# jacky121298/3DAL_PyTorch

Measured on AMD Instinct MI355X. Metric: object-crops/sec through static+dynamic refinement heads, higher is better.
Workload: dtype f32; 1 GPU; StaticModelOneBoxEst forward+decode, 4096 crops x 1024 pts per GPU, fp32 (BASELINE.json configs[1]); items_per_gpu=4096, points_per_item=1024, sampler=device, parallelism=single GPU

## Files before the change

3dal_pytorch_amd/_hip.py:

```python
import ctypes as C
import os

import numpy as np
import torch

_HERE = os.path.dirname(os.path.abspath(__file__))
LIB_PATH = os.path.join(_HERE, "lib3dal_hip.so")

OK, EINVAL, EWORKSPACE, EHIP = 0, -1, -2, -3
F32, BF16, F16, F16X3 = 0, 1, 2, 3
DTYPES = {"fp32": F32, "bf16": BF16, "fp16": F16, "f16x3": F16X3}
HEAD_INS_SEG, HEAD_STATIC_BOX_EST, HEAD_POINT_EMB, HEAD_BOX_EMB, HEAD_DYNAMIC_BOX_EST = range(5)
SAMPLER_DEVICE, SAMPLER_CHOICE = 0, 1
PHASE_SEG, PHASE_BOX, PHASE_ALL = 1, 2, 3

vp = C.c_void_p


class Layer(C.Structure):
    _fields_ = [("weight", vp), ("bias", vp), ("bn_weight", vp), ("bn_bias", vp), ("bn_mean", vp),
                ("bn_var", vp), ("c_in", C.c_int32), ("c_out", C.c_int32)]


class PackItem(C.Structure):
# ... 246 lines not shown
    _fields_ = [("c_in", C.c_int32), ("n_shared", C.c_int32), ("n_cls", C.c_int32), ("n_reg", C.c_int32), ("shared", _i3),
                ("cls", _i3), ("reg", _i3), ("num_class", C.c_int32), ("code_size", C.c_int32)]


class RoiHeadArgs(C.Structure):
    _fields_ = [("shape", RoiShape), ("packed", vp), ("B", C.c_int64), ("M", C.c_int64), ("num_point", C.c_int32), ("C", C.c_int32),
                ("T", C.c_int32), ("box_cols", C.c_int32), ("K", C.c_int64), ("keep_stride", C.c_int64), ("boxes", vp), ("scores", vp),
                ("labels", vp), ("keep", vp), ("keep_count", vp), ("seg_offsets", vp), ("label_base", C.c_int32 * ROI_MAX_TASKS),
                ("bev", Map), ("H", C.c_int64), ("W", C.c_int64), ("pc_start", _f2), ("voxel_size", _f2), ("out_stride", C.c_float),
                ("rois", vp), ("roi_scores", vp), ("roi_features", vp), ("out_boxes", vp), ("out_scores", vp), ("out_labels", vp),
                ("out_counts", vp), ("out_features", vp), ("box_preds", vp), ("cls_preds", vp), ("status", vp), ("workspace", vp),
                ("workspace_bytes", C.c_size_t)]


ROI_NO_SAMPLE = 8192
ROI_CLS_SCORE = {"roi_iou": 0, "cls": 1}
ROI_TRAIN_MAX_M, ROI_TRAIN_MAX_R, ROI_TRAIN_MAX_G = 512, 512, 1024


class RoiTargetsArgs(C.Structure):
    _fields_ = [("B", C.c_int64), ("M", C.c_int64), ("R", C.c_int64), ("G", C.c_int64), ("code_size", C.c_int32),
                ("reserved0", C.c_int32), ("T", C.c_int32), ("reserved", C.c_int32), ("K", C.c_int64), ("keep_stride", C.c_int64),
                ("boxes", vp), ("scores", vp), ("labels", vp), ("keep", vp), ("keep_count", vp), ("seg_offsets", vp),
                ("label_base", C.c_int32 * ROI_MAX_TASKS), ("rois", vp), ("roi_scores", vp), ("roi_labels", vp), ("gt", vp),
                ("draws", vp), ("fg_per_image", C.c_int32), ("cls_score_type", C.c_int32), ("reg_fg_thresh", C.c_float),
                ("cls_fg_thresh", C.c_float), ("cls_bg_thresh", C.c_float), ("cls_bg_thresh_lo", C.c_float),
                ("cls_thresh_span", C.c_float), ("reserved2", C.c_float), ("hard_bg_ratio", C.c_double), ("slot", vp), ("sample", vp),
                ("out_rois", vp), ("out_labels", vp), ("out_scores", vp), ("gt_iou", vp), ("gt_src", vp), ("reg_valid", vp),
                ("cls_labels", vp), ("gt_of_rois", vp), ("out_boxes", vp), ("status", vp)]


CENTER_OVERFLOW = 16384
CENTER_MAX_OBJS, CENTER_MAX_CLASSES, CENTER_MAX_COLS = 1024, 64, 10
_pT = vp * ROI_MAX_TASKS


class CenterTargetsArgs(C.Structure):
    _fields_ = [("B", C.c_int64), ("G", C.c_int64), ("H", C.c_int64), ("W", C.c_int64), ("T", C.c_int32), ("max_objs", C.c_int32),
                ("num_class", C.c_int32 * ROI_MAX_TASKS), ("gt", vp), ("pc_start", _f2), ("voxel_size", _f2),
                ("out_size_factor", C.c_float), ("min_radius", C.c_int32), ("gaussian_overlap", C.c_double), ("hm", _pT),
                ("anno_box", _pT), ("ind", _pT), ("mask", _pT), ("cat", _pT), ("status", vp)]


class CenterLossArgs(C.Structure):
    _fields_ = [("B", C.c_int64), ("H", C.c_int64), ("W", C.c_int64), ("C", C.c_int32), ("n_cols", C.c_int32), ("max_objs", C.c_int32),
                ("reserved", C.c_int32), ("hm", Map), ("reg", Map), ("height", Map), ("dim", Map), ("rot", Map), ("vel", Map),
                ("target_hm", vp), ("anno_box", vp), ("ind", vp), ("mask", vp), ("cat", vp),
                ("code_weights", C.c_float * CENTER_MAX_COLS), ("weight", C.c_float), ("reserved2", C.c_float), ("out", vp),
                ("grad", vp), ("workspace", vp), ("workspace_bytes", C.c_size_t)]


AUG_TOO_MANY, AUG_OVERFLOW, AUG_BAD_ROW = 32768, 65536, 131072
AUG_MAX_BOXES, AUG_MAX_CAND = 1024, 64


class GtPasteArgs(C.Structure):
    _fields_ = [("B", C.c_int64), ("max_gt", C.c_int32), ("max_cand", C.c_int32), ("gt_boxes", vp), ("gt_classes", vp),
                ("gt_counts", vp), ("cand_boxes", vp), ("cand_group", vp), ("cand_counts", vp), ("accept", vp), ("coll", vp),
                ("status", vp)]


class AugmentPointsArgs(C.Structure):
    _fields_ = [("B", C.c_int64), ("n", C.c_int64), ("n_scene", C.c_int64), ("db_rows", C.c_int64), ("F", C.c_int32),
                ("transform", C.c_int32), ("max_cand", C.c_int64), ("scene", vp), ("scene_offsets", vp), ("db_points", vp),
                ("out_offsets", vp), ("cand_counts", vp), ("cand_seg_start", vp), ("cand_rows", vp), ("cand_db_row", vp),
                ("cand_boxes", vp), ("accept", vp), ("keys", vp), ("xform", vp), ("out", vp), ("status", vp),
                ("max_workgroups", C.c_int64), ("workspace", vp), ("workspace_bytes", C.c_size_t)]


class AugmentBoxesArgs(C.Structure):
    _fields_ = [("B", C.c_int64), ("max_gt", C.c_int32), ("max_cand", C.c_int32), ("max_objs", C.c_int32), ("n_classes", C.c_int32),
                ("transform", C.c_int32), ("reserved", C.c_int32), ("gt_boxes", vp), ("gt_classes", vp), ("gt_counts", vp),
                ("cand_boxes", vp), ("cand_classes", vp), ("cand_counts", vp), ("accept", vp), ("xform", vp),
                ("range", C.c_float * 4), ("out", vp), ("out_count", vp), ("status", vp)]


_i, _i64, _u64, _sz = C.c_int, C.c_int64, C.c_uint64, C.c_size_t
SIGNATURES = {
    "dal3_version": (_i, []),
    "dal3_last_error": (C.c_char_p, []),
    "dal3_mean_size": (C.POINTER(C.c_float), []),
    "dal3_pack_weights": (_i, [_i, C.POINTER(Layer), _i, _i, vp, C.POINTER(_sz), vp]),
    "dal3_ins_seg_workspace_bytes": (_sz, [_i]),
    "dal3_ins_seg_forward": (_i, [vp, _i, _i, BCN, _i, _i, vp, vp, vp, vp, _sz, vp]),
    "dal3_ins_seg_encode": (_i, [vp, _i, _i, BCN, _i, _i, vp, vp]),
    "dal3_ins_seg_global_bias": (_i, [vp, _i, vp, _i, vp, vp]),
    "dal3_ins_seg_decode": (_i, [vp, _i, _i, BCN, _i, _i, vp, vp, vp, vp]),
    "dal3_gather_workspace_bytes": (_sz, [_i, _i]),
    "dal3_segment_counts": (_i, [vp, _i, _i, vp, vp]),
    "dal3_mask_compact_sample": (_i, [vp, BCN, _i, _i, _i, _i, _i, vp, _u64, _i64, vp, vp, vp, vp, _sz, vp]),
    "dal3_mask_compact_sample_step": (_i, [vp, BCN, _i, _i, _i, _i, _u64, vp, _i64, vp, vp, vp, vp, _sz, vp]),
    "dal3_point_head_workspace_bytes": (_sz, [_i]),
    "dal3_point_head_forward": (_i, [_i, vp, _i, BCN, _i, _i, vp, _i64, vp, _sz, vp]),
    "dal3_point_head_pool_workspace_bytes": (_sz, [_i, _i]),
    "dal3_point_head_screen_min_tiles": (_i, []),
    "dal3_point_head_screen_stride": (_i, []),
    "dal3_point_head_pool": (_i, [_i, vp, _i, BCN, _i, _i, vp, vp, vp, _sz, vp]),
    "dal3_dynamic_box_est_forward": (_i, [vp, vp, _i, vp, vp, _sz, vp]),
    "dal3_decode_boxes": (_i, [vp, _i, vp, _i64, _i, vp, _i64, vp, _i64, vp, vp, vp, vp, vp]),
    "dal3_recenter_rotz": (_i, [vp, _i, _i, vp, vp, vp, vp, vp, vp, vp]),
    "dal3_static_crop_prep": (_i, [vp, vp, vp, vp, vp, _i, _i, _u64, _i64, vp, vp, vp]),
    "dal3_dynamic_item_prep": (_i, [vp, vp, vp, vp, vp, vp, vp, vp, _i, _i, _i, _i, _u64, _i64, vp, vp, vp, vp]),
    "dal3_writeback_boxes": (_i, [vp, vp, vp, vp, vp, vp, vp, vp, vp, _i, _i64, vp, vp, vp]),
    "dal3_static_crop_labels": (_i, [vp, vp, vp, vp, _i, _i, _u64, _i64, vp, vp, vp]),
    "dal3_dynamic_item_labels": (_i, [vp, vp, vp, vp, vp, vp, vp, _i, _i, _i, _u64, _i64, vp, vp, vp, vp, vp]),
    "dal3_points_in_boxes": (_i, [vp, _i, _i64, _i64, vp, _i, _i, vp, vp]),
    "dal3_box_iou_pairwise": (_i, [vp, _i64, vp, _i64, _i, vp, vp, vp]),
    "dal3_box_iou_paired": (_i, [vp, vp, _i64, _i, vp, vp, vp]),
    "dal3_box_estimation_metrics": (_i, [C.POINTER(BoxMetricArgs), vp]),
    "dal3_track_workspace_bytes": (_sz, [_i64, _i64, _i64]),
    "dal3_track": (_i, [C.POINTER(TrackArgs), vp]),
    "dal3_track_match_workspace_bytes": (_sz, [_i64]),
    "dal3_track_match": (_i, [C.POINTER(TrackMatchArgs), vp]),
    "dal3_group_workspace_bytes": (_sz, [_i64, _i64]),
    "dal3_group_by_key": (_i, [C.POINTER(GroupArgs), vp]),
    "dal3_track_features": (_i, [C.POINTER(TrackFeatureArgs), vp]),
    "dal3_gt_table": (_i, [C.POINTER(GtTableArgs), vp]),
    "dal3_motion_classify_workspace_bytes": (_sz, [_i64]),
    "dal3_motion_classify": (_i, [C.POINTER(MotionClassifyArgs), vp]),
    "dal3_score_workspace_bytes": (_sz, [_i64]),
    "dal3_score_tracks": (_i, [C.POINTER(ScoreArgs), vp]),
    "dal3_best_gt_iou": (_i, [C.POINTER(BestGtArgs), vp]),
    "dal3_nms_workspace_bytes": (_sz, [_i64, _i]),
    "dal3_nms": (_i, [C.POINTER(NmsArgs), vp]),
    "dal3_center_decode_workspace_bytes": (_sz, [_i64, _i64, _i64]),
    "dal3_center_decode": (_i, [C.POINTER(CenterDecodeArgs), vp]),
    "dal3_center_decode_flip4_workspace_bytes": (_sz, [_i64, _i64, _i64]),
    "dal3_center_decode_flip4": (_i, [C.POINTER(CenterDecodeFlip4Args), vp]),
    "dal3_flip4_points": (_i, [vp, _i64, C.c_int32, vp, _i64, vp, vp, _i64, vp]),
    "dal3_voxelize_workspace_bytes": (_sz, [_i64, _i64]),
    "dal3_voxelize": (_i, [C.POINTER(VoxelizeArgs), vp]),
    "dal3_pillar_pack": (_i, [C.POINTER(Layer), _i, _i, C.c_double, vp, vp]),
    "dal3_pillar_features": (_i, [C.POINTER(PillarFeatureArgs), vp]),
    "dal3_pillar_scatter": (_i, [vp, vp, _i64, vp, _i, vp, _i64, _i64, _i64, vp]),
    "dal3_voxel_mean": (_i, [vp, vp, _i64, vp, _i, _i, vp, vp]),
    "dal3_conv2d_pack_floats": (_sz, [_i, _i, _i]),
    "dal3_conv2d_pack": (_i, [C.POINTER(Layer), _i, C.c_double, vp, vp]),
    "dal3_conv2d": (_i, [C.POINTER(Conv2dArgs), vp]),
    "dal3_sp_sort_workspace_bytes": (_sz, [_i64]),
    "dal3_sp_sort": (_i, [C.POINTER(SpSortArgs), vp]),
    "dal3_sp_downsample_workspace_bytes": (_sz, [_i64, _i]),
    "dal3_sp_downsample": (_i, [C.POINTER(SpDownsampleArgs), vp]),
    "dal3_sp_table": (_i, [C.POINTER(SpTableArgs), vp]),
    "dal3_sp_conv_pack_floats": (_sz, [_i, _i, _i]),
    "dal3_sp_conv_pack": (_i, [C.POINTER(Layer), _i, C.c_double, vp, vp, vp]),
    "dal3_sp_conv": (_i, [C.POINTER(SpConvArgs), vp]),
    "dal3_sp_table_transposed": (_i, [C.POINTER(SpTableTransposedArgs), vp]),
    "dal3_sp_wgrad_workspace_bytes": (_sz, [_i, _i, _i, _i64]),
    "dal3_sp_wgrad": (_i, [C.POINTER(SpWgradArgs), vp]),
    "dal3_bev_gather": (_i, [C.POINTER(BevGatherArgs), vp]),
    "dal3_box_points": (_i, [vp, _i64, _i, _i, vp, vp]),
    "dal3_roi_pack_floats": (_sz, [C.POINTER(RoiShape)]),
    "dal3_roi_pack": (_i, [C.POINTER(RoiShape), C.POINTER(Layer), _i, C.POINTER(C.c_double), vp, vp]),
    "dal3_roi_head_workspace_bytes": (_sz, [_i64, _i64, _i, _i, _i]),
    "dal3_roi_head": (_i, [C.POINTER(RoiHeadArgs), vp]),
    "dal3_roi_post": (_i, [vp, vp, vp, _i64, _i, vp, vp, vp]),
    "dal3_roi_targets": (_i, [C.POINTER(RoiTargetsArgs), vp]),
    "dal3_roi_loss": (_i, [vp, vp, _i64, _i, vp, vp, vp, C.POINTER(C.c_float), C.c_float, C.c_float, vp, vp, vp, vp]),
    "dal3_center_targets": (_i, [C.POINTER(CenterTargetsArgs), vp]),
    "dal3_center_loss_workspace_bytes": (_sz, [_i64, _i64, _i64, _i64]),
    "dal3_center_loss": (_i, [C.POINTER(CenterLossArgs), vp]),
    "dal3_gt_paste_select": (_i, [C.POINTER(GtPasteArgs), vp]),
    "dal3_augment_points_workspace_bytes": (_sz, [_i64, _i64]),
    "dal3_augment_points": (_i, [C.POINTER(AugmentPointsArgs), vp]),
    "dal3_augment_boxes": (_i, [C.POINTER(AugmentBoxesArgs), vp]),
    "dal3_crop_workspace_bytes": (_sz, [_i64, _i64]),
# ... 60 lines not shown
    "dal3_tr_wgrad_x3": (_i, [vp, _i64, vp, _i64, vp, vp, _i, vp, _i64, _i, _i, vp, _sz, vp, vp]),
    "dal3_tr_segmax": (_i, [vp, _i64, _i64, _i, vp, vp, vp, vp, _i64, vp, _sz, vp]),
    "dal3_tr_act_dropout": (_i, [vp, _i64, _i, _i64, vp, vp, _i, vp, _i64, _u64, vp, C.c_float, vp, _i64, vp]),
    "dal3_tr_linear_pool_workspace_bytes": (_sz, [_i, _i, _i64]),
    "dal3_tr_linear_pool": (_i, [vp, _i64, _i, _i64, vp, vp, _i, vp, _i64, vp, vp, vp, _i64, _i, vp, vp, vp, _sz, vp]),
    "dal3_tr_linear_pool_x3": (_i, [vp, _i64, _i, _i64, vp, vp, _i, vp, _i64, vp, vp, vp, _i64, _i, vp, vp, vp, _sz, vp]),
    "dal3_tr_linear_pool_x3_ok": (_i, [_i64, _i, _i64, _i]),
    "dal3_tr_segsum": (_i, [vp, _i64, _i64, _i, vp, _i64, vp]),
    "dal3_maxpool_n": (_i, [vp, _i64, _i64, vp, vp]),
    "dal3_maxpool_n_dtype": (_i, [vp, _i, _i64, _i64, vp, vp]),
    "dal3_shared_mlp_layer": (_i, [C.POINTER(Layer), _i, BCN, _i, _i, vp, vp, _sz, vp]),
    "dal3_shared_mlp_layer_workspace_bytes": (_sz, [_i, _i]),
    "dal3_static_workspace_bytes": (_sz, [_i, _i, _i]),
    "dal3_static_forward": (_i, [C.POINTER(StaticArgs), _i, vp]),
    "dal3_dynamic_workspace_bytes": (_sz, [_i, _i, _i]),
    "dal3_dynamic_forward": (_i, [C.POINTER(DynamicArgs), _i, vp]),
}

_lib = None


def lib():
    global _lib
    if _lib is None:
        if not os.path.exists(LIB_PATH):
            raise RuntimeError(
                f"{LIB_PATH} is missing: build the HIP library first "
                "(`make -C 3dal_pytorch_amd/csrc` or __graft_entry__.build()). "
                "There is no CPU/eager fallback for the eval-mode forward.")
        handle = C.CDLL(LIB_PATH)
        for name, (res, args) in SIGNATURES.items():
            fn = getattr(handle, name)
            fn.restype = res
            fn.argtypes = args
        from . import arch
        lib_mean = [handle.dal3_mean_size()[i] for i in range(9)]
        want = [C.c_float(v).value for row in arch.MEAN_SIZE for v in row]
        if lib_mean != want:
            raise RuntimeError(f"lib3dal_hip.so was built with MEAN_SIZE {lib_mean}, arch.MEAN_SIZE is {want}: rebuild the library")
        _lib = handle
    return _lib


def check(rc):
    if rc != OK:
        raise RuntimeError(f"lib3dal_hip error {rc}: {lib().dal3_last_error().decode()}")


def stream():
    return vp(torch.cuda.current_stream().cuda_stream)


def ptr(t):
    return vp(t.data_ptr()) if t is not None else vp(None)


def require_gpu(t, what):
    if not t.is_cuda:
        raise RuntimeError(
            f"{what} lives on {t.device}: the eval-mode forward runs only on an MI355X through "
            "lib3dal_hip.so (no CPU fallback). Move the model and its inputs to the GPU.")


def workspace(nbytes, device):
    return torch.empty(max(int(nbytes), 8), dtype=torch.uint8, device=device)


def host_offsets(offsets, n, name, sized_by, count):
    if torch.is_tensor(offsets):
        if offsets.is_cuda:
            raise TypeError(f"{name} must be on the host (a list, an array or a CPU tensor): {sized_by} from it, and "
                            "reading a device tensor back would be the synchronisation this call avoids")
        offsets = offsets.numpy()
    off = np.ascontiguousarray(np.asarray(offsets, dtype=np.int64).reshape(-1))
    if off.size < 1:
        raise ValueError(f"{name} needs {count} + 1 entries")
    if off[0] < 0 or off[-1] > n or np.any(np.diff(off) < 0):
        raise ValueError(f"{name} must be non-decreasing within [0, {n}]")
    return off


STORAGE = {torch.float32: F32, torch.bfloat16: BF16, torch.float16: F16}
BCN_NO_SMALL_JOB_KERNELS, BCN_NO_WORKLIST, BCN_NO_LDS_SAMPLER = 1, 2, 4
DISPATCH_FLAGS = 0


def bcn(t):
    assert t.dim() == 3 and t.dtype in STORAGE
    sb, sc, sn = t.stride()
    return BCN(ptr(t), sb, sc, sn, STORAGE[t.dtype], DISPATCH_FLAGS)


def layer_struct(conv, bn):
    w = conv.weight
    c_in, c_out = getattr(conv, "in_channels", w.shape[1]), getattr(conv, "out_channels", w.shape[0])
    if not w.is_contiguous() or w.dtype != torch.float32:
        raise RuntimeError("weights must be contiguous fp32")
    L = Layer(ptr(w), ptr(conv.bias), None, None, None, None, c_in, c_out)
    if bn is not None:
        L.bn_weight, L.bn_bias = ptr(bn.weight), ptr(bn.bias)
        L.bn_mean, L.bn_var = ptr(bn.running_mean), ptr(bn.running_var)
    return L


def fold_layer_struct(conv, bn, what="the layer's parameters"):
    ts = [conv.weight] + ([conv.bias] if conv.bias is not None else [])
    if bn is not None:
        ts += [bn.weight, bn.bias, bn.running_mean, bn.running_var]
    for t in ts:
        require_gpu(t, what)
        if t.dtype != torch.float32 or not t.is_contiguous():
            raise RuntimeError("weights must be contiguous fp32")
    return layer_struct(conv, bn)


F16_MAX = 65504.0


def check_f16x3_range(pairs):
    with torch.no_grad():
        worst = None
        for conv, bn in pairs:
            w = conv.weight.detach().reshape(conv.weight.shape[0], -1).abs().amax(1)
            if bn is not None:
                w = w * (bn.weight.detach() / torch.sqrt(bn.running_var.detach() + 1e-5)).abs()
            m = w.max()
            worst = m if worst is None else torch.maximum(worst, m)
        if worst is not None and not float(worst) < F16_MAX:
            raise ValueError(f"precision 'f16x3': a folded weight of magnitude {float(worst):.3g} is beyond fp16's range "
                             f"({F16_MAX:g}); this head cannot run on the f16x3 kernels (use precision 'fp32')")


def pack(head_kind, pairs, device, dtype=F32):
    if dtype == F16X3:
        check_f16x3_range(pairs)
    arr = (Layer * len(pairs))(*[layer_struct(c, b) for c, b in pairs])
    need = _sz(0)
    check(lib().dal3_pack_weights(head_kind, arr, len(pairs), dtype, None, C.byref(need), None))
    buf = torch.empty(need.value, dtype=torch.uint8, device=device)
    assert buf.data_ptr() % 256 == 0
    check(lib().dal3_pack_weights(head_kind, arr, len(pairs), dtype, ptr(buf), C.byref(need), stream()))
    return buf
```

3dal_pytorch_amd/csrc/dal3_api.hip:

```cpp
#include <stdarg.h>
#include <stdio.h>
#include <string.h>

#include "dal3_block.h"
#include "dal3_kernels.h"
#include "dal3_lp.h"

static thread_local char g_err[512] = "";

static int fail(int code, const char* fmt, ...) {
    va_list ap;
    va_start(ap, fmt);
    vsnprintf(g_err, sizeof(g_err), fmt, ap);
    va_end(ap);
    return code;
}

#define HIP_TRY(expr)                                                                           \
    do {                                                                                        \
        hipError_t e_ = (expr);                                                                 \
        if (e_ != hipSuccess) return fail(DAL3_EHIP, "%s: %s", #expr, hipGetErrorString(e_)); \
    } while (0)
#define TRY(expr)               \
    do {                        \
        int r_ = (expr);        \
        if (r_ != 0) return r_; \
    } while (0)

extern "C" int dal3_version(void) { return DAL3_VERSION; }
extern "C" const float* dal3_mean_size(void) {
    static const float v[9] = {DAL3_MEAN_SIZE_VALUES};
    return v;
}
extern "C" const char* dal3_last_error(void) { return g_err; }

static inline size_t al(size_t floats) { return (floats + 63) & ~(size_t)63; }

struct Cursor {
    const float* base;
    size_t off;
    const float* take(size_t floats) {
        const float* p = base ? base + off : nullptr;
        off += al(floats);
        return p;
    }
    const f32x4* take4(size_t floats) { return reinterpret_cast<const f32x4*>(take(floats)); }
};

static InsSegW ins_seg_walk(Cursor& c) {
    InsSegW w;
    w.w1 = c.take(2 * 2 * 64);
    w.b1 = c.take(64);    w.b2 = c.take(64);    w.b3 = c.take(64);    w.b4 = c.take(128);   w.b5 = c.take(1024);
    w.dw1g = c.take(512 * 1024);
    w.db1 = c.take(512);  w.db2 = c.take(256);  w.db3 = c.take(128);  w.db4 = c.take(128);
    w.dw5 = c.take(2 * 128);
    w.db5 = c.take(32);
    w.enc_stream = c.take4((size_t)ENC_FRAGS * 256);
    w.dec_stream = c.take4((size_t)DEC_FRAGS * 256);
    w.lat_stream = c.take4((size_t)LAT_FRAGS * 256);
    w.w5row = c.take((size_t)1024 * 128);
    w.w5h = c.take4((size_t)32 * 4 * 2 * 256);
    w.scr_pq = c.take(2 * 1024);
    w.scr_flag = reinterpret_cast<const int32_t*>(c.take(64));
    w.dw2c = c.take((size_t)512 * 256);
    w.dw3c = c.take((size_t)256 * 128);
    w.dw4c = c.take((size_t)128 * 128);
    w.dec_flag = reinterpret_cast<const int32_t*>(c.take(64));
    return w;
}

size_t ins_seg_packed_floats(int) {
    Cursor c{nullptr, 0};
    ins_seg_walk(c);
    return c.off + DAL3_BLOB_TAIL_FLOATS;
}
InsSegW ins_seg_view(const float* base, int) {
    Cursor c{base, 0};
    return ins_seg_walk(c);
}

void point_head_dims(int head_kind, int* c_in, int* ks, int c[4], int* n_fc, int fc_in[3], int fc_out[3]) {
    switch (head_kind) {
        case DAL3_HEAD_STATIC_BOX_EST:
            *c_in = 3; *ks = 2; c[0] = 128; c[1] = 128; c[2] = 256; c[3] = 512; *n_fc = 3;
            fc_in[0] = 512; fc_out[0] = 512; fc_in[1] = 512; fc_out[1] = 256; fc_in[2] = 256; fc_out[2] = 39;
            break;
        case DAL3_HEAD_POINT_EMB:
            *c_in = 4; *ks = 2; c[0] = 64; c[1] = 128; c[2] = 256; c[3] = 512; *n_fc = 2;
            fc_in[0] = 512; fc_out[0] = 512; fc_in[1] = 512; fc_out[1] = 256; fc_in[2] = 0; fc_out[2] = 0;
            break;
        default:
            *c_in = 8; *ks = 4; c[0] = 64; c[1] = 64; c[2] = 128; c[3] = 512; *n_fc = 2;
            fc_in[0] = 512; fc_out[0] = 128; fc_in[1] = 128; fc_out[1] = 128; fc_in[2] = 0; fc_out[2] = 0;
            break;
    }
}

static PointHeadW point_head_walk(Cursor& cur, int head_kind) {
    int c_in, ks, c[4], n_fc, fi[3], fo[3];
    point_head_dims(head_kind, &c_in, &ks, c, &n_fc, fi, fo);
    PointHeadW w;
    w.w1 = cur.take((size_t)(c[0] / 32) * ks * 64);
    w.b1 = cur.take(c[0]);    w.b2 = cur.take(c[1]);    w.b3 = cur.take(c[2]);    w.b4 = cur.take(c[3]);
    w.stream = cur.take4(((size_t)(c[1] / 32) * (c[0] / 32) + (size_t)(c[2] / 32) * (c[1] / 32) +
                          (size_t)(c[3] / 32) * (c[2] / 32)) * 1024);
    w.fc.n = n_fc;
    for (int i = 0; i < 3; ++i) {
        w.fc.c_in[i] = fi[i];
        w.fc.c_out[i] = fo[i];
        w.fc.relu[i] = !(head_kind == DAL3_HEAD_STATIC_BOX_EST && i == 2);
        w.fc.w[i] = i < n_fc ? cur.take((size_t)fi[i] * fo[i]) : nullptr;
        w.fc.b[i] = i < n_fc ? cur.take((fo[i] + 31) / 32 * 32) : nullptr;
    }
    const bool scr = c[2] == 256 && c[3] == 512;
    w.w4row = scr ? cur.take((size_t)512 * 256) : nullptr;
    w.w4h = scr ? cur.take4((size_t)16 * 8 * 2 * 256) : nullptr;
    w.scr_pq = scr ? cur.take(2 * 512) : nullptr;
    w.scr_flag = scr ? reinterpret_cast<const int32_t*>(cur.take(64)) : nullptr;
    return w;
}
size_t point_head_packed_floats(int head_kind) {
    Cursor c{nullptr, 0};
    point_head_walk(c, head_kind);
    return c.off + DAL3_BLOB_TAIL_FLOATS;
}
PointHeadW point_head_view(const float* base, int head_kind) {
    Cursor c{base, 0};
    return point_head_walk(c, head_kind);
}

static const int kDynFcIn[3] = {384, 128, 128}, kDynFcOut[3] = {128, 128, 39};
static FcW fc_head_walk(Cursor& cur) {
    FcW f;
    f.n = 3;
    for (int i = 0; i < 3; ++i) {
        f.c_in[i] = kDynFcIn[i];
        f.c_out[i] = kDynFcOut[i];
        f.relu[i] = i < 2;
        f.w[i] = cur.take((size_t)kDynFcIn[i] * kDynFcOut[i]);
        f.b[i] = cur.take((kDynFcOut[i] + 31) / 32 * 32);
    }
    return f;
}
size_t fc_head_packed_floats() {
    Cursor c{nullptr, 0};
    fc_head_walk(c);
    return c.off;
}
FcW fc_head_view(const float* base) {
// ... 187 lines not shown
            HIP_TRY(launch_pack_weight(L[0], PACK_FIRST, 0, c_in, 2, 2, mut(w.w1), s));
            HIP_TRY(launch_pack_bias(L[0], mut(w.b1), s));
            HIP_TRY(launch_pack_bias(L[1], be, s));
            HIP_TRY(launch_pack_bias(L[2], be + 64, s));
            HIP_TRY(launch_pack_bias(L[3], be + 128, s));
            HIP_TRY(launch_pack_bias(L[4], be + 256, s));
            HIP_TRY(launch_pack_bias(L[1], bd, s));
            HIP_TRY(launch_pack_bias(L[6], bd + 64, s));
            HIP_TRY(launch_pack_bias(L[7], bd + 320, s));
            HIP_TRY(launch_pack_bias(L[8], bd + 448, s));
            HIP_TRY(launch_pack_bias(L[9], bd + 576, s));
            HIP_TRY(launch_pack_weight(L[5], PACK_ROWMAJOR, 64, 1024, 0, 0, mut(w.dw1g), s));
            HIP_TRY(launch_pack_bias(L[5], mut(w.db1), s));
            HIP_TRY(launch_pack_weight_x3(L[1], 0, 0, 64, 2, 2, enc, s));
            HIP_TRY(launch_pack_weight_x3(L[2], 0, 0, 64, 2, 2, enc + 16 * F, s));
            HIP_TRY(launch_pack_weight_x3(L[3], 0, 0, 64, 4, 2, enc + 32 * F, s));
            HIP_TRY(launch_pack_weight_x3(L[4], 0, 0, 128, 32, 4, enc + 64 * F, s));
            HIP_TRY(launch_pack_weight_x3(L[1], 0, 0, 64, 2, 2, dec, s));
            HIP_TRY(launch_pack_weight_x3(L[5], 0, 0, 64, 16, 2, dec, s, 2, 16 * F, 24 * F, 40 * F));
            HIP_TRY(launch_pack_weight_x3(L[6], 1, 0, 512, 8, 16, dec, s, 8, 32 * F, 72 * F, 40 * F, 624 * F));
            HIP_TRY(launch_pack_weight_x3(L[7], 0, 0, 256, 4, 8, dec + 656 * F, s));
            HIP_TRY(launch_pack_weight_x3(L[8], 0, 0, 128, 4, 4, dec + 784 * F, s));
            HIP_TRY(launch_pack_weight_x3(L[9], 0, 0, 128, 1, 4, dec + 848 * F, s));
            return 0;
        }
        if (lp) {
            const InsSegLpW w = ins_seg_lp_view(packed_dev);
            uint16_t* enc = const_cast<uint16_t*>(w.enc_stream);
            uint16_t* dec = const_cast<uint16_t*>(w.dec_stream);
            float* be = mut(w.bias_enc);
            float* bd = mut(w.bias_dec);
            const int64_t F = 512;
            HIP_TRY(launch_pack_weight(L[0], PACK_FIRST, 0, c_in, 2, 2, mut(w.w1), s));
            HIP_TRY(launch_pack_bias(L[0], mut(w.b1), s));
            HIP_TRY(launch_pack_bias(L[1], be, s));
            HIP_TRY(launch_pack_bias(L[2], be + 64, s));
            HIP_TRY(launch_pack_bias(L[3], be + 128, s));
            HIP_TRY(launch_pack_bias(L[4], be + 256, s));
            HIP_TRY(launch_pack_bias(L[1], bd, s));
            HIP_TRY(launch_pack_bias(L[6], bd + 64, s));
            HIP_TRY(launch_pack_bias(L[7], bd + 320, s));
            HIP_TRY(launch_pack_bias(L[8], bd + 448, s));
            HIP_TRY(launch_pack_weight(L[9], PACK_ROWMAJOR, 0, 128, 0, 0, bd + 576, s));
            HIP_TRY(launch_pack_bias(L[9], bd + 832, s));
            HIP_TRY(launch_pack_weight(L[5], PACK_ROWMAJOR, 64, 1024, 0, 0, mut(w.dw1g), s));
            HIP_TRY(launch_pack_bias(L[5], mut(w.db1), s));
            HIP_TRY(launch_pack_weight_lp(L[1], dtype, 0, 0, 64, 2, 2, enc, s));
            HIP_TRY(launch_pack_weight_lp(L[2], dtype, 0, 0, 64, 2, 2, enc + 8 * F, s));
            HIP_TRY(launch_pack_weight_lp(L[3], dtype, 0, 0, 64, 4, 2, enc + 16 * F, s));
            HIP_TRY(launch_pack_weight_lp(L[4], dtype, 0, 0, 128, 32, 4, enc + 32 * F, s));
            HIP_TRY(launch_pack_weight_lp(L[1], dtype, 0, 0, 64, 2, 2, dec, s));
            HIP_TRY(launch_pack_weight_lp(L[5], dtype, 0, 0, 64, 16, 2, dec, s, 2, 8 * F, 40 * F, 20 * F));
            HIP_TRY(launch_pack_weight_lp(L[6], dtype, 1, 0, 512, 8, 16, dec, s, 8, 44 * F, 64 * F, 20 * F));
            HIP_TRY(launch_pack_weight_lp(L[7], dtype, 0, 0, 256, 4, 8, dec, s, 16, 360 * F, 400 * F, 40 * F));
            HIP_TRY(launch_pack_weight_lp(L[8], dtype, 0, 0, 128, 4, 4, dec + 440 * F, s));
            HIP_TRY(launch_pack_weight_lp(L[9], dtype, 0, 0, 128, 1, 4, dec + 472 * F, s));
            return 0;
        }
        InsSegW w = ins_seg_view(base, c_in);
        HIP_TRY(launch_pack_weight(L[0], PACK_FIRST, 0, c_in, 2, 2, mut(w.w1), s));
        HIP_TRY(launch_pack_bias(L[0], mut(w.b1), s));
        TRY(pack_frag(L[1], PACK_FRAG_MT_MAJOR, 0, 64, w.enc_stream, ENC_W2, w.b2, s));
        TRY(pack_frag(L[2], PACK_FRAG_MT_MAJOR, 0, 64, w.enc_stream, ENC_W3, w.b3, s));
        TRY(pack_frag(L[3], PACK_FRAG_MT_MAJOR, 0, 64, w.enc_stream, ENC_W4, w.b4, s));
        TRY(pack_frag(L[4], PACK_FRAG_MT_MAJOR, 0, 128, w.enc_stream, ENC_W5, w.b5, s));
        TRY(pack_frag(L[1], PACK_FRAG_MT_MAJOR, 0, 64, w.dec_stream, DEC_W2, nullptr, s));
        TRY(pack_frag(L[5], PACK_FRAG_MT_MAJOR, 0, 64, w.dec_stream, DEC_MIX, w.db1, s,  2,
                      0, 8 * 256, 40 * 256));
        HIP_TRY(launch_pack_weight(L[5], PACK_ROWMAJOR, 64, 1024, 0, 0, mut(w.dw1g), s));
        TRY(pack_frag(L[6], PACK_FRAG_KT_MAJOR, 0, 512, w.dec_stream, DEC_MIX, w.db2, s,  8,
                      16 * 256, 56 * 256, 40 * 256));
        TRY(pack_frag(L[7], PACK_FRAG_MT_MAJOR, 0, 256, w.dec_stream, DEC_W3, w.db3, s));
        TRY(pack_frag(L[8], PACK_FRAG_MT_MAJOR, 0, 128, w.dec_stream, DEC_W4, w.db4, s));
        TRY(pack_frag(L[5], PACK_FRAG_MT_MAJOR, 0, 64, w.lat_stream, LAT_W1A, nullptr, s));
        TRY(pack_frag(L[6], PACK_FRAG_MT_MAJOR, 0, 512, w.lat_stream, LAT_W2, nullptr, s));
        HIP_TRY(launch_pack_weight(L[9], PACK_ROWMAJOR, 0, 128, 0, 0, mut(w.dw5), s));
        HIP_TRY(launch_pack_bias(L[9], mut(w.db5), s));
        HIP_TRY(launch_pack_weight(L[4], PACK_ROWMAJOR, 0, 128, 0, 0, mut(w.w5row), s));
        HIP_TRY(launch_pack_weight_lp(L[4], DAL3_F16, 0, 0, 128, 32, 4, reinterpret_cast<uint16_t*>(mut(w.w5h)), s));
        HIP_TRY(launch_pack_enc_screen(L[4], mut(w.scr_pq), reinterpret_cast<int32_t*>(mut(w.scr_flag)), s));
        HIP_TRY(launch_pack_dec_sparse(L[6], w.db2, mut(w.dw2c), reinterpret_cast<int32_t*>(const_cast<int32_t*>(w.dec_flag)), s));
        HIP_TRY(launch_pack_dec_queue(L[7], 256, w.db3, mut(w.dw3c), reinterpret_cast<int32_t*>(const_cast<int32_t*>(w.dec_flag)), s));
        HIP_TRY(launch_pack_dec_queue(L[8], 128, w.db4, mut(w.dw4c), reinterpret_cast<int32_t*>(const_cast<int32_t*>(w.dec_flag)), s));
        return 0;
    }
    if (head_kind == DAL3_HEAD_DYNAMIC_BOX_EST) {
        if (n_layers != 3) return fail(DAL3_EINVAL, "dynamic box_est expects 3 layers, got %d", n_layers);
        return pack_fc(L, fc_head_view(base), s);
    }
    int c_in, ks, c[4], n_fc, fi[3], fo[3];
    point_head_dims(head_kind, &c_in, &ks, c, &n_fc, fi, fo);
    if (n_layers != 4 + n_fc) return fail(DAL3_EINVAL, "head %d expects %d layers, got %d", head_kind, 4 + n_fc, n_layers);
    TRY(check_layer(L[0], c_in, c[0], "conv1"));
    for (int i = 1; i < 4; ++i) TRY(check_layer(L[i], c[i - 1], c[i], "conv"));
    if (x3) {
        const PointHeadX3W w = point_head_x3_view(packed_dev, head_kind);
        HIP_TRY(launch_pack_weight(L[0], PACK_FIRST, 0, c_in, c[0] / 32, ks, mut(w.w1), s));
        HIP_TRY(launch_pack_bias(L[0], mut(w.b1), s));
        HIP_TRY(launch_pack_bias(L[1], mut(w.bias), s));
        HIP_TRY(launch_pack_bias(L[2], mut(w.bias) + c[1], s));
        HIP_TRY(launch_pack_bias(L[3], mut(w.bias) + c[1] + c[2], s));
        uint16_t* st = const_cast<uint16_t*>(w.stream);
        int64_t off = 0;
        for (int l = 1; l < 4; ++l) {
            const int kt = c[l - 1] / 32, mt = c[l] / 32;
            HIP_TRY(launch_pack_weight_x3(L[l], 0, 0, c[l - 1], mt, kt, st + off, s));
            off += (int64_t)mt * kt * 2048;
        }
        return pack_fc(L + 4, w.fc, s);
    }
    if (lp) {
        const PointHeadLpW w = point_head_lp_view(packed_dev, head_kind);
        HIP_TRY(launch_pack_weight(L[0], PACK_FIRST, 0, c_in, c[0] / 32, ks, mut(w.w1), s));
        HIP_TRY(launch_pack_bias(L[0], mut(w.b1), s));
        HIP_TRY(launch_pack_bias(L[1], mut(w.bias), s));
        HIP_TRY(launch_pack_bias(L[2], mut(w.bias) + c[1], s));
        HIP_TRY(launch_pack_bias(L[3], mut(w.bias) + c[1] + c[2], s));
        uint16_t* st = const_cast<uint16_t*>(w.stream);
        const int64_t SEGE = (int64_t)LP_HEAD_SEG * 512;
        int seg = 0;
        for (int l = 1; l < 4; ++l) {
            const int kt = c[l - 1] / 32, mt = c[l] / 32, tps = lp_tps(kt, mt);
            HIP_TRY(launch_pack_weight_lp(L[l], dtype, 0, 0, c[l - 1], mt, kt, st, s, tps * kt, seg * SEGE,
                                          (seg + 1) * SEGE, SEGE));
            seg += mt / tps;
        }
        return pack_fc(L + 4, w.fc, s);
    }
    PointHeadW w = point_head_view(base, head_kind);
    HIP_TRY(launch_pack_weight(L[0], PACK_FIRST, 0, c_in, c[0] / 32, ks, mut(w.w1), s));
    HIP_TRY(launch_pack_bias(L[0], mut(w.b1), s));
    const int f3 = (c[1] / 32) * (c[0] / 32) * 4, f4 = f3 + (c[2] / 32) * (c[1] / 32) * 4;
    TRY(pack_frag(L[1], PACK_FRAG_MT_MAJOR, 0, c[0], w.stream, 0, w.b2, s));
    TRY(pack_frag(L[2], PACK_FRAG_MT_MAJOR, 0, c[1], w.stream, f3, w.b3, s));
    TRY(pack_frag(L[3], PACK_FRAG_MT_MAJOR, 0, c[2], w.stream, f4, w.b4, s));
    if (w.w4row) {
        HIP_TRY(launch_pack_weight(L[3], PACK_ROWMAJOR, 0, 256, 0, 0, mut(w.w4row), s));
        HIP_TRY(launch_pack_weight_lp(L[3], DAL3_F16, 0, 0, 256, 16, 8, reinterpret_cast<uint16_t*>(mut(w.w4h)), s));
        HIP_TRY(launch_pack_head_screen(L[3], mut(w.scr_pq), reinterpret_cast<int32_t*>(mut(w.scr_flag)), s));
    }
    return pack_fc(L + 4, w.fc, s);
}

static BCN to_bcn(const dal3_bcn& t) { return BCN{t.data, t.stride_b, t.stride_c, t.stride_n, t.dtype, t.flags}; }

static int check_bcn(const dal3_bcn& t, const char* what) {
    if (!t.data) return fail(DAL3_EINVAL, "%s: null data pointer", what);
    if (t.stride_n <= 0 || t.stride_c <= 0) return fail(DAL3_EINVAL, "%s: strides must be positive", what);
    if (t.dtype != DAL3_F32 && t.dtype != DAL3_BF16 && t.dtype != DAL3_F16)
        return fail(DAL3_EINVAL, "%s: storage dtype %d is none of DAL3_F32 / DAL3_BF16 / DAL3_F16", what, t.dtype);
    if (t.dtype != DAL3_F32 && (reinterpret_cast<uintptr_t>(t.data) & 1)) return fail(DAL3_EINVAL, "%s: 16-bit data must be 2-byte aligned", what);
    if (t.flags & ~(DAL3_BCN_NO_SMALL_JOB_KERNELS | DAL3_BCN_NO_WORKLIST | DAL3_BCN_NO_LDS_SAMPLER)) return fail(DAL3_EINVAL, "%s: unknown bits in flags (%d)", what, t.flags);
    return 0;
}

static int check_extent(int64_t B, int64_t N, const char* what) {
    if (B <= 0 || N <= 0) return fail(DAL3_EINVAL, "%s: B and N must be positive (B=%lld N=%lld)", what, (long long)B, (long long)N);
    if (B > DAL3_MAX_ITEMS) return fail(DAL3_EINVAL, "%s: B=%lld items exceed DAL3_MAX_ITEMS (%d)", what, (long long)B, DAL3_MAX_ITEMS);
    if (N > DAL3_MAX_POINTS_PER_ITEM)
        return fail(DAL3_EINVAL, "%s: N=%lld points per item exceed DAL3_MAX_POINTS_PER_ITEM (%d)", what, (long long)N, DAL3_MAX_POINTS_PER_ITEM);
    if (B * ((N + 31) / 32) > (int64_t)DAL3_MAX_TILES)
        return fail(DAL3_EINVAL, "%s: B=%lld x N=%lld is %lld 32-point tiles, more than DAL3_MAX_TILES (%d): split the batch", what,
                    (long long)B, (long long)N, (long long)(B * ((N + 31) / 32)), DAL3_MAX_TILES);
    return 0;
}

struct InsSegWs { float* g; float* gb; };
static InsSegWs carve_ins_seg(Carver& c, int B) {
    InsSegWs w;
    w.g = c.take<float>((size_t)B * 1024);
    w.gb = c.take<float>((size_t)B * 512);
    return w;
}
extern "C" size_t dal3_ins_seg_workspace_bytes(int B) {
    Carver c(nullptr, 0);
    carve_ins_seg(c, B);
    return c.off;
}

static int check_dtype(int dtype) {
    if (dtype != DAL3_F32 && dtype != DAL3_BF16 && dtype != DAL3_F16 && dtype != DAL3_F16X3)
        return fail(DAL3_EINVAL, "unknown dtype %d", dtype);
    return 0;
}

static int ins_seg_run(const void* packed, int dtype, int c_in, const dal3_bcn& pts, int B, int N, float* logits,
                       uint8_t* mask, float* global_feat_out, const InsSegWs& ws, hipStream_t s) {
    TRY(check_dtype(dtype));
    if (!packed || !logits || !mask) return fail(DAL3_EINVAL, "ins_seg: null pointer");
    TRY(check_extent(B, N, "ins_seg"));
    if (c_in != 3 && c_in != 4) return fail(DAL3_EINVAL, "ins_seg: c_in must be 3 or 4");
    TRY(check_bcn(pts, "pts"));
    const BCN x = to_bcn(pts);
    HIP_TRY(launch_nonfinite_rows(x, B, N, c_in, ws.g, 1024, s));
    if (dtype == DAL3_F32) {
        const InsSegW w = ins_seg_view(static_cast<const float*>(packed), c_in);
        HIP_TRY(launch_ins_seg_encode(w, x, c_in, B, N, ws.g, s));
        HIP_TRY(launch_fc(w.dw1g, w.db1, ws.g, 1024, ws.gb, 512, B, 1024, 512, 0, s));
        HIP_TRY(launch_ins_seg_decode(w, x, c_in, B, N, ws.gb, logits, mask, s));
    } else if (dtype == DAL3_F16X3) {
        const InsSegX3W w = ins_seg_x3_view(packed);
        HIP_TRY(launch_ins_seg_encode_x3(w, x, c_in, B, N, ws.g, s));
        HIP_TRY(launch_fc(w.dw1g, w.db1, ws.g, 1024, ws.gb, 512, B, 1024, 512, 0, s));
        HIP_TRY(launch_ins_seg_decode_x3(w, x, c_in, B, N, ws.gb, logits, mask, s));
    } else {
        const InsSegLpW w = ins_seg_lp_view(packed);
        HIP_TRY(launch_ins_seg_encode_lp(dtype, w, x, c_in, B, N, ws.g, s));
        HIP_TRY(launch_fc(w.dw1g, w.db1, ws.g, 1024, ws.gb, 512, B, 1024, 512, 0, s));
        HIP_TRY(launch_ins_seg_decode_lp(dtype, w, x, c_in, B, N, ws.gb, logits, mask, s));
    }
    if (global_feat_out)
        HIP_TRY(hipMemcpyAsync(global_feat_out, ws.g, (size_t)B * 1024 * sizeof(float), hipMemcpyDeviceToDevice, s));
    return 0;
}

extern "C" int dal3_ins_seg_forward(const void* packed, int dtype, int c_in, dal3_bcn pts, int B, int N, float* logits,
                                    uint8_t* mask, float* global_feat_out, void* workspace, size_t workspace_bytes,
                                    dal3_stream stream) {
    if (!workspace) return fail(DAL3_EINVAL, "ins_seg: workspace is NULL");
    TRY(check_extent(B, N, "ins_seg"));
    Carver c(workspace, workspace_bytes);
    const InsSegWs ws = carve_ins_seg(c, B);
    if (!c.ok) return fail(DAL3_EWORKSPACE, "ins_seg: workspace needs %zu bytes, got %zu", c.off, workspace_bytes);
    return ins_seg_run(packed, dtype, c_in, pts, B, N, logits, mask, global_feat_out, ws, static_cast<hipStream_t>(stream));
}

extern "C" int dal3_ins_seg_encode(const void* packed, int dtype, int c_in, dal3_bcn pts, int B, int N,
                                   float* global_feat, dal3_stream stream) {
    TRY(check_dtype(dtype));
    if (!packed || !global_feat || (c_in != 3 && c_in != 4)) return fail(DAL3_EINVAL, "ins_seg_encode: bad argument");
    TRY(check_extent(B, N, "ins_seg_encode"));
    TRY(check_bcn(pts, "pts"));
    hipStream_t s = static_cast<hipStream_t>(stream);
    if (dtype == DAL3_F32)
        HIP_TRY(launch_ins_seg_encode(ins_seg_view(static_cast<const float*>(packed), c_in), to_bcn(pts), c_in, B, N,
                                      global_feat, s));
    else if (dtype == DAL3_F16X3)
        HIP_TRY(launch_ins_seg_encode_x3(ins_seg_x3_view(packed), to_bcn(pts), c_in, B, N, global_feat, s));
    else
        HIP_TRY(launch_ins_seg_encode_lp(dtype, ins_seg_lp_view(packed), to_bcn(pts), c_in, B, N, global_feat, s));
    return 0;
}

extern "C" int dal3_ins_seg_global_bias(const void* packed, int dtype, const float* global_feat, int B, float* gbias,
                                        dal3_stream stream) {
    TRY(check_dtype(dtype));
    if (!packed || !global_feat || !gbias) return fail(DAL3_EINVAL, "ins_seg_global_bias: bad argument");
    TRY(check_extent(B, 1, "ins_seg_global_bias"));
    const float* dw1g = dtype == DAL3_F32 ? ins_seg_view(static_cast<const float*>(packed), 3).dw1g
                        : dtype == DAL3_F16X3 ? ins_seg_x3_view(packed).dw1g : ins_seg_lp_view(packed).dw1g;
    const float* db1 = dtype == DAL3_F32 ? ins_seg_view(static_cast<const float*>(packed), 3).db1
                       : dtype == DAL3_F16X3 ? ins_seg_x3_view(packed).db1 : ins_seg_lp_view(packed).db1;
    HIP_TRY(launch_fc(dw1g, db1, global_feat, 1024, gbias, 512, B, 1024, 512, 0, static_cast<hipStream_t>(stream)));
    return 0;
}

extern "C" int dal3_ins_seg_decode(const void* packed, int dtype, int c_in, dal3_bcn pts, int B, int N,
                                   const float* gbias, float* logits, uint8_t* mask, dal3_stream stream) {
    TRY(check_dtype(dtype));
    if (!packed || !gbias || !logits || !mask || (c_in != 3 && c_in != 4)) return fail(DAL3_EINVAL, "ins_seg_decode: bad argument");
    TRY(check_extent(B, N, "ins_seg_decode"));
    TRY(check_bcn(pts, "pts"));
    hipStream_t s = static_cast<hipStream_t>(stream);
    if (dtype == DAL3_F32)
        HIP_TRY(launch_ins_seg_decode(ins_seg_view(static_cast<const float*>(packed), c_in), to_bcn(pts), c_in, B, N,
                                      gbias, logits, mask, s));
    else if (dtype == DAL3_F16X3)
        HIP_TRY(launch_ins_seg_decode_x3(ins_seg_x3_view(packed), to_bcn(pts), c_in, B, N, gbias, logits, mask, s));
    else
        HIP_TRY(launch_ins_seg_decode_lp(dtype, ins_seg_lp_view(packed), to_bcn(pts), c_in, B, N, gbias, logits, mask, s));
    return 0;
}

extern "C" size_t dal3_gather_workspace_bytes(int B, int N) {
    Carver c(nullptr, 0);
    c.take<int32_t>((size_t)B * N);
    return c.off;
}

extern "C" int dal3_segment_counts(const uint8_t* mask, int B, int N, int32_t* counts, dal3_stream stream) {
    if (!mask || !counts) return fail(DAL3_EINVAL, "segment_counts: bad argument");
    TRY(check_extent(B, N, "segment_counts"));
// ... 1985 lines not shown
```

3dal_pytorch_amd/csrc/dal3_enc_screen.hip:

```cpp
#include "dal3_device.h"
#include "dal3_kernels.h"
#include "dal3_lp.h"
#include "dal3_screen.h"

#ifndef SCR_CAP
#define SCR_CAP 1024
#endif
#define SCR_XLD 132
#define SCR_STAGE_LD 36
#ifndef SCR_DEPTH
#define SCR_DEPTH 2
#endif
#define SCR_XMAX_BITS 0x476A6000
#ifndef DAL3_SCR_A_STRIDE
#define DAL3_SCR_A_STRIDE 4
#endif
static_assert(DAL3_SCR_A_STRIDE >= 1, "pass A's stride over the wave-slots");

#ifdef DAL3_SCREEN_COUNT
__device__ unsigned long long g_scr_count[8];
extern "C" int dal3_debug_screen_counts(unsigned long long* out, int reset) {
    hipError_t e = hipMemcpyFromSymbol(out, HIP_SYMBOL(g_scr_count), sizeof(g_scr_count));
    if (e == hipSuccess && reset) {
        unsigned long long z[8] = {};
        e = hipMemcpyToSymbol(HIP_SYMBOL(g_scr_count), z, sizeof(z));
    }
    return (int)e;
}
#define SCR_COUNT(k, v)                                           \
    do {                                                          \
        if (lane == 0) atomicAdd(&g_scr_count[k], (unsigned long long)(v)); \
    } while (0)
#else
#define SCR_COUNT(k, v)
#endif

template <int PASS, int T>
__global__ __launch_bounds__(64 * DAL3_WG_WAVES) void ins_seg_encode_screen_kernel(InsSegW w, BCN pts, int c_in, int n_pts,
                                                                                  int tiles_per_item, float* __restrict__ g) {
    const int lane = threadIdx.x & 63;
    const int wave = threadIdx.x >> 6;
    const int h = lane >> 5;
    const int64_t b = blockIdx.x / tiles_per_item;
    const int n0 = ((blockIdx.x % tiles_per_item) * DAL3_WG_WAVES + wave) * (PASS == 0 ? DAL3_SCR_A_STRIDE : 1) * (32 * T);
    __shared__ float s_b5[1024];
    __shared__ int s_max[1024];
    __shared__ f32x2 s_pq[1024];
    __shared__ float s_g[PASS == 1 ? 1024 : 1];
    __shared__ __attribute__((aligned(16))) float s_x[PASS == 1 ? DAL3_WG_WAVES * 32 * SCR_XLD : 4];
    __shared__ uint32_t s_list[PASS == 1 ? DAL3_WG_WAVES * T * SCR_CAP : 1];
    __shared__ __attribute__((aligned(16))) uint32_t s_stage[PASS == 1 ? DAL3_WG_WAVES * 64 * SCR_STAGE_LD : 4];
    int* gi = reinterpret_cast<int*>(g + b * 1024);
    static_assert(20 * 1024 + DAL3_WG_WAVES * (32 * SCR_XLD * 4 + T * SCR_CAP * 4 + 64 * SCR_STAGE_LD * 4) <= 160 * 1024,
                  "pass B's LDS exceeds a CU's 160 KiB: lower SCR_CAP, DAL3_WG_WAVES or DAL3_ENC_T");
    static_assert(32 * 64 <= 64 * SCR_STAGE_LD, "a wave's stage holds the hit words of conv5's 32 blocks");
    if (PASS == 0 && *w.scr_flag != 0) return;
    for (int i = threadIdx.x; i < 1024; i += 64 * DAL3_WG_WAVES) {
        s_b5[i] = w.b5[i];
        s_max[i] = 0;
        s_pq[i] = reinterpret_cast<const f32x2*>(w.scr_pq)[i];
        if (PASS == 1) s_g[i] = __int_as_float(__hip_atomic_load(gi + i, __ATOMIC_RELAXED, __HIP_MEMORY_SCOPE_AGENT));
    }
    __syncthreads();
    if (n0 < n_pts) {
        WRing<DAL3_PF> ring;
        ring.init(w.enc_stream, lane);
        f32x16 bias = tile_from_channels(w.b2, h);
        float in[T][2];
        load_points<2, T>(pts, b, n0, n_pts, c_in, in, lane);
        f32x16 x1[T][2], x2[T][2], x3[T][2], x4[T][4];
        first_layer<2, 2, T>(w.w1, w.b1, in, x1, lane);
        mlp_layer_ring<2, 2, T>(ring, w.b2, w.b3, bias, x1, x2, lane);
        mlp_layer_ring<2, 2, T>(ring, w.b3, w.b4, bias, x2, x3, lane);
        mlp_layer_ring<2, 4, T>(ring, w.b4, w.b4, bias, x3, x4, lane);
        SCR_COUNT(0, 1);

        int xm = 0;
#pragma unroll
        for (int j = 0; j < T; ++j) {
#pragma unroll
            for (int kt = 0; kt < 4; ++kt) {
#pragma unroll
                for (int r = 0; r < 16; ++r) {
                    const int v = __float_as_int(x4[j][kt][r]);
                    xm = v > xm ? v : xm;
                }
            }
        }
        const bool dense = *w.scr_flag != 0 || __builtin_amdgcn_ballot_w64(xm > SCR_XMAX_BITS) != 0;
        if (dense) {
            SCR_COUNT(1, 1);
            if (PASS == 1) conv_max_layer<4, T>(ring, s_b5, x4, reinterpret_cast<float*>(s_max), 32, lane);
        } else {
            float x2max = 0.0f;
#pragma unroll
            for (int j = 0; j < T; ++j) {
                float ss = 0.0f;
#pragma unroll
                for (int kt = 0; kt < 4; ++kt) {
#pragma unroll
                    for (int r = 0; r < 16; ++r) ss = fmaf(x4[j][kt][r], x4[j][kt][r], ss);
                }
                ss += __shfl_xor(ss, 32);
                x2max = __builtin_fmaxf(x2max, ss);
            }
#pragma unroll
            for (int d = 16; d >= 1; d >>= 1) x2max = __builtin_fmaxf(x2max, __shfl_xor(x2max, d));
            const float X = sqrtf(x2max) * (1.0f + 0x1p-16f);

            ActTile<FP16> xh[T][4];
#pragma unroll
            for (int j = 0; j < T; ++j) {
#pragma unroll
                for (int kt = 0; kt < 4; ++kt) xh[j][kt] = pack_relu<FP16>(x4[j][kt]);
            }

            uint32_t* const list = s_list + (PASS == 1 ? wave * T * SCR_CAP : 0);
            uint32_t* const stage = s_stage + (PASS == 1 ? wave * 64 * SCR_STAGE_LD : 0);
            ScreenHits<T> hits;
            hits.init();

            auto block_const = [&](int mt) -> float {
                const int c = 32 * mt + (lane & 31);
                const f32x2 pq = s_pq[c];
                float E = fmaf(X, pq[0], pq[1]);
                E = fmaf(E, 0x1p-20f, E);
                if (PASS == 0) return E;
                const float G = s_g[c], bb = s_b5[c];
                if (bits_nonfinite(G)) return 3.0e38f;
                return (G - bb) - fmaf(__builtin_fabsf(G) + __builtin_fabsf(bb), 0x1p-22f, E);
            };
            static_assert(16 * T <= 32, "one hit bit per (tile, register) in a 32-bit word");
            float m = 0.0f;
            uint32_t hb = 0;
            auto ep_slice = [&](const f32x16 (&acc)[T], int i, float k) {
#pragma unroll
                for (int rr = 0; rr < 2; ++rr) {
#pragma unroll
                    for (int j = 0; j < T; ++j) {
                        const int r = 2 * i + rr;
                        if (PASS == 0)
                            m = (r == 0 && j == 0) ? acc[0][0] : __builtin_fmaxf(m, acc[j][r]);
                        else
                            hb = scr_push_hit(hb, acc[j][r], k);
                    }
                }
            };
            auto ep_finish = [&](int mt, float k) {
                const int c = 32 * mt + (lane & 31);
                if (PASS == 0) {
                    m = __builtin_fmaxf(m, __shfl_xor(m, 32));
                    const float y = m - fmaf(__builtin_fabsf(m), 0x1p-22f, k);
                    int bits = __float_as_int(y + s_b5[c]);
                    bits = bits > 0 ? bits : 0;
                    if (lane < 32 && bits > 0) atomicMax(&s_max[c], bits);
// ... 3 lines not shown
            };

            WRing<8> r16;
            r16.init(w.w5h, lane);
            auto mm = [&](f32x16 (&acc)[T], auto side) {
#pragma unroll
                for (int j = 0; j < T; ++j) acc[j] = f32x16{};
#pragma unroll
                for (int i = 0; i < 8; ++i) {
                    const f16x8_t a = __builtin_bit_cast(f16x8_t, r16.slot[i]);
                    r16.slot[i] = r16.fetch();
#pragma unroll
                    for (int j = 0; j < T; ++j) acc[j] = FP16::mfma(xh[j][i >> 1].k[i & 1], a, acc[j]);
                    DAL3_SCHED_FENCE();
                    side(i);
                    DAL3_SCHED_FENCE();
                }
            };
            f32x16 accA[T], accB[T];
            float kA = block_const(0), kB;
            mm(accA, NoSide());
            int mt = 1;
            for (; mt + 1 < 32; mt += 2) {
                kB = block_const(mt);
                mm(accB, [&](int i) { ep_slice(accA, i, kA); });
                ep_finish(mt - 1, kA);
                kA = block_const(mt + 1);
                mm(accA, [&](int i) { ep_slice(accB, i, kB); });
                ep_finish(mt, kB);
            }
            kB = block_const(mt);
            mm(accB, [&](int i) { ep_slice(accA, i, kA); });
            ep_finish(mt - 1, kA);
#pragma unroll
            for (int i = 0; i < 8; ++i) ep_slice(accB, i, kB);
            ep_finish(mt, kB);

            if (PASS == 1) {
                uint32_t cnt[T];
                const bool overflow = scr_build_lists<T, 32, SCR_CAP>(stage, list, hits, cnt, lane);
#pragma unroll
                for (int j = 0; j < T; ++j) SCR_COUNT(3, cnt[j]);
                if (overflow) {
                    SCR_COUNT(2, 1);
                    WRing<DAL3_PF> r32;
                    r32.init(w.enc_stream + ENC_W5 * 64, lane);
                    conv_max_layer<4, T>(r32, s_b5, x4, reinterpret_cast<float*>(s_max), 32, lane);
                } else {
                    float* const xw = s_x + wave * 32 * SCR_XLD;
#pragma unroll
                    for (int j = 0; j < T; ++j) {
                        __builtin_amdgcn_wave_barrier();
#pragma unroll
                        for (int kt = 0; kt < 4; ++kt) {
#pragma unroll
                            for (int q = 0; q < 4; ++q) {
                                f32x4 v;
                                v[0] = x4[j][kt][4 * q + 0];
                                v[1] = x4[j][kt][4 * q + 1];
                                v[2] = x4[j][kt][4 * q + 2];
                                v[3] = x4[j][kt][4 * q + 3];
                                *reinterpret_cast<f32x4*>(xw + (lane & 31) * SCR_XLD + 32 * kt + 8 * q + 4 * h) = v;
                            }
                        }
                        __builtin_amdgcn_wave_barrier();
                        SCR_COUNT(4, (cnt[j] + 63) / 64);
                        scr_recompute<32, 4, SCR_DEPTH, true>(
                            w.w5row, 128, list + j * SCR_CAP, cnt[j], xw, SCR_XLD, stage, lane, [](uint32_t, bool) { return 0.0f; },
                            [&](float a, int c, uint32_t, bool live) {
                                int bits = __float_as_int(a + s_b5[c]);
                                bits = bits > 0 ? bits : 0;
                                if (live && bits > 0) atomicMax(&s_max[c], bits);
                            });
                    }
                }
            }
        }
    }
    __syncthreads();
    for (int c = threadIdx.x; c < 1024; c += 64 * DAL3_WG_WAVES) {
        const int v = s_max[c];
        if (v > 0) atomicMax(gi + c, v);
    }
}

hipError_t launch_ins_seg_encode_screen(const InsSegW& w, BCN pts, int c_in, int B, int N, float* g, hipStream_t s) {
    constexpr int T = DAL3_ENC_T;
    const int tpi = (N + 32 * DAL3_WG_WAVES * T - 1) / (32 * DAL3_WG_WAVES * T);
    const int slots = (N + 32 * T - 1) / (32 * T);
    const int tpi_a = ((slots + DAL3_SCR_A_STRIDE - 1) / DAL3_SCR_A_STRIDE + DAL3_WG_WAVES - 1) / DAL3_WG_WAVES;
    const dim3 grid_a((unsigned)((int64_t)B * tpi_a)), grid((unsigned)((int64_t)B * tpi)), block(64 * DAL3_WG_WAVES);
    hipLaunchKernelGGL((ins_seg_encode_screen_kernel<0, T>), grid_a, block, 0, s, w, pts, c_in, N, tpi_a, g);
    hipError_t e = hipGetLastError();
    if (e != hipSuccess) return e;
    hipLaunchKernelGGL((ins_seg_encode_screen_kernel<1, T>), grid, block, 0, s, w, pts, c_in, N, tpi, g);
    return hipGetLastError();
}
```

3dal_pytorch_amd/csrc/dal3_kernels.h:

```cpp
#pragma once
#include <hip/hip_runtime.h>
#include <stddef.h>
#include <stdint.h>

#include "../../include/dal3.h"
#include "dal3_device.h"
#include "dal3_fold.h"

#ifndef DAL3_ENC_T
#define DAL3_ENC_T 2
#endif
#ifndef DAL3_DEC_T
#define DAL3_DEC_T 1
#endif
#ifndef DAL3_HEAD_T
#define DAL3_HEAD_T 1
#endif

#ifndef DAL3_ENC_SCREEN
#define DAL3_ENC_SCREEN 1
#endif

#ifndef DAL3_WG_WAVES
#define DAL3_WG_WAVES 4
#endif

#ifndef DAL3_PF
#define DAL3_PF 8
#endif
#define DAL3_MEAN_SIZE_VALUES 4.8, 1.8, 1.5, 10.0, 2.6, 3.2, 2.0, 1.0, 1.6
__device__ __forceinline__ double mean_size_f64(int sc, int j) {
    constexpr double m[9] = {DAL3_MEAN_SIZE_VALUES};
    return sc == 0 ? (j == 0 ? m[0] : j == 1 ? m[1] : m[2])
                   : sc == 1 ? (j == 0 ? m[3] : j == 1 ? m[4] : m[5]) : (j == 0 ? m[6] : j == 1 ? m[7] : m[8]);
}
#define DAL3_BLOB_TAIL_FLOATS 8192

struct InsSegW {
    const float* w1;
    const float* b1;
    const float* b2;
    const float* b3;
    const float* b4;
    const float* b5;
    const float* dw1g;
    const float* db1;
    const float* db2;
    const float* db3;
    const float* db4;
    const float* dw5;
    const float* db5;
    const f32x4* enc_stream;
    const f32x4* dec_stream;
    const f32x4* lat_stream;
    const float* w5row;
    const f32x4* w5h;
    const float* scr_pq;
    const int32_t* scr_flag;
    const float* dw2c;
    const float* dw3c;
    const float* dw4c;
    const int32_t* dec_flag;
};
enum {
    ENC_W2 = 0, ENC_W3 = 16, ENC_W4 = 32, ENC_W5 = 64, ENC_FRAGS = 64 + 512,
    DEC_W2 = 0, DEC_MIX = 16, DEC_MIX_FRAGS = 8 + 16 * 40, DEC_W3 = 16 + 648, DEC_W4 = 16 + 648 + 128,
    DEC_FRAGS = 16 + 648 + 128 + 64,
    LAT_W1A = 0, LAT_W2 = 128, LAT_FRAGS = 128 + 512
};

struct FcW {
    const float* w[3];
    const float* b[3];
    int c_in[3], c_out[3], relu[3];
    int n;
};

struct PointHeadW {
    const float* w1;
    const float* b1;
    const float* b2;
    const float* b3;
    const float* b4;
    const f32x4* stream;
    FcW fc;
    const float* w4row;
    const f32x4* w4h;
    const float* scr_pq;
    const int32_t* scr_flag;
};

#define LP_ENC_SEG 32
#define LP_ENC_SEGS 9
#define LP_DEC_SEG 40
#define LP_DEC_SEGS 12
#define LP_HEAD_SEG 32
#ifndef DAL3_LP_ENC_T
#define DAL3_LP_ENC_T 4
#endif
#ifndef DAL3_LP_DEC_T
#define DAL3_LP_DEC_T 2
#endif
#ifndef DAL3_LP_HEAD_T
#define DAL3_LP_HEAD_T 2
#endif
struct InsSegLpW {
    const float* w1;
    const float* b1;
    const float* bias_enc;
    const float* bias_dec;
    const float* dw1g;
    const float* db1;
    const uint16_t* enc_stream;
    const uint16_t* dec_stream;
};
struct PointHeadLpW {
    const float* w1;
    const float* b1;
    const float* bias;
    const uint16_t* stream;
    FcW fc;
};
#ifndef DAL3_X3_HEAD_T
#define DAL3_X3_HEAD_T 2
#endif
#ifndef DAL3_X3_ENC_T
#define DAL3_X3_ENC_T 2
#endif
#ifndef DAL3_X3_DEC_T
#define DAL3_X3_DEC_T 2
#endif
typedef PointHeadLpW PointHeadX3W;
struct InsSegX3W {
    const float* w1;
    const float* b1;
    const float* bias_enc;
    const float* bias_dec;
    const float* dw1g;
    const float* db1;
    const uint16_t* enc_stream;
    const uint16_t* dec_stream;
};
size_t ins_seg_x3_packed_bytes();
InsSegX3W ins_seg_x3_view(const void* base);
hipError_t launch_ins_seg_encode_x3(const InsSegX3W& w, BCN pts, int c_in, int B, int N, float* g, hipStream_t s);
hipError_t launch_ins_seg_decode_x3(const InsSegX3W& w, BCN pts, int c_in, int B, int N, const float* gbias, float* logits,
                                    uint8_t* mask, hipStream_t s);
size_t point_head_x3_packed_bytes(int head_kind);
PointHeadX3W point_head_x3_view(const void* base, int head_kind);
int point_head_x3_segments(int head_kind);
hipError_t launch_point_head_x3(int head_kind, const PointHeadX3W& w, BCN x, int c_in, int B, int M, float* feat,
                                const int32_t* distinct, hipStream_t s);
hipError_t launch_pack_weight_x3(const dal3_layer& L, int kt_major, int col_off, int n_cols, int mt_n, int kt_n, uint16_t* out,
                                 hipStream_t s, int grp_blocks = 0, int64_t grp_a0 = 0, int64_t grp_a1 = 0,
                                 int64_t grp_stride = 0, int64_t grp_last = -1);
size_t ins_seg_lp_packed_bytes();
InsSegLpW ins_seg_lp_view(const void* base);
size_t point_head_lp_packed_bytes(int head_kind);
PointHeadLpW point_head_lp_view(const void* base, int head_kind);
int point_head_lp_segments(int head_kind);
hipError_t launch_ins_seg_encode_lp(int dtype, const InsSegLpW& w, BCN pts, int c_in, int B, int N, float* g, hipStream_t s);
hipError_t launch_ins_seg_decode_lp(int dtype, const InsSegLpW& w, BCN pts, int c_in, int B, int N, const float* gbias,
                                    float* logits, uint8_t* mask, hipStream_t s);
hipError_t launch_point_head_lp(int dtype, int head_kind, const PointHeadLpW& w, BCN x, int c_in, int B, int M,
                                float* feat, const int32_t* distinct, hipStream_t s);
hipError_t launch_pack_weight_lp(const dal3_layer& L, int dtype, int kt_major, int col_off, int n_cols, int mt_n, int kt_n,
                                 uint16_t* out, hipStream_t s, int grp_blocks = 0, int64_t grp_a0 = 0, int64_t grp_a1 = 0,
                                 int64_t grp_stride = 0);

size_t ins_seg_packed_floats(int c_in);
InsSegW ins_seg_view(const float* base, int c_in);
size_t point_head_packed_floats(int head_kind);
PointHeadW point_head_view(const float* base, int head_kind);
size_t fc_head_packed_floats();
FcW fc_head_view(const float* base);
void point_head_dims(int head_kind, int* c_in, int* ks, int c[4], int* n_fc, int fc_in[3], int fc_out[3]);

hipError_t launch_ins_seg_encode(const InsSegW& w, BCN pts, int c_in, int B, int N, float* g, hipStream_t s);
hipError_t launch_ins_seg_encode_screen(const InsSegW& w, BCN pts, int c_in, int B, int N, float* g, hipStream_t s);
hipError_t launch_pack_enc_screen(const dal3_layer& L, float* pq, int32_t* flag, hipStream_t s);
hipError_t launch_pack_dec_sparse(const dal3_layer& L, const float* db2, float* dw2c, int32_t* flag, hipStream_t s);
hipError_t launch_pack_dec_queue(const dal3_layer& L, int c_in, const float* bias, float* wcopy, int32_t* flag, hipStream_t s);
hipError_t launch_ins_seg_decode(const InsSegW& w, BCN pts, int c_in, int B, int N, const float* gbias,
                                 float* logits, uint8_t* mask, hipStream_t s);
size_t point_head_worklist_bytes(int B, int M);
hipError_t launch_point_head(int head_kind, const PointHeadW& w, BCN x, int c_in, int B, int M, float* feat,
                             const int32_t* distinct, hipStream_t s, void* worklist = nullptr, size_t worklist_bytes = 0);
#ifndef DAL3_HEAD_SCR_STRIDE
#define DAL3_HEAD_SCR_STRIDE 4
#endif
#ifndef DAL3_HEAD_SCREEN
#define DAL3_HEAD_SCREEN 1
#endif
#ifndef DAL3_HEAD_SCR_MIN_TILES
#define DAL3_HEAD_SCR_MIN_TILES 8192
#endif
static_assert(DAL3_HEAD_SCR_STRIDE >= 2, "stride 1 leaves no tile to screen");
hipError_t launch_point_head_screen(int head_kind, const PointHeadW& w, BCN x, int c_in, float* feat, uint32_t* ctl,
                                    const u32x4* list, int64_t max_tiles, int64_t slots, hipStream_t s);
hipError_t launch_pack_head_screen(const dal3_layer& L, float* pq, int32_t* flag, hipStream_t s);
hipError_t launch_generic_layer(const f32x4* wf, const float* w1, const float* bias, int kt_n, int ks_n, int mt_n,
                                int relu, BCN x, int c_in, int B, int N, float* y, hipStream_t s);

hipError_t launch_fc(const float* W, const float* bias, const float* x, int64_t xs, float* y, int64_t ys, int B,
                     int c_in, int c_out, int relu, hipStream_t s);

enum { PACK_FRAG_MT_MAJOR = 0, PACK_FRAG_KT_MAJOR = 1, PACK_FIRST = 2, PACK_ROWMAJOR = 3 };
hipError_t launch_pack_weight(const dal3_layer& L, int mode, int col_off, int n_cols, int mt_n, int kt_n, float* out,
                              hipStream_t s, int grp_blocks = 0, int64_t grp_a0 = 0, int64_t grp_a1 = 0,
                              int64_t grp_stride = 0);
hipError_t launch_pack_bias(const dal3_layer& L, float* out, hipStream_t s);

hipError_t launch_static_crop_prep(const double* points, const int64_t* offsets, const int32_t* choice, const double* pose,
                                   const double* box, int B, int N, uint64_t seed, int64_t item_offset, float* pts_out,
                                   float* init_box_out, hipStream_t s);
hipError_t launch_dynamic_item_prep(const double* points, const int64_t* frame_offsets, const double* boxes,
                                    const int64_t* track_first, const int32_t* item_track, const int32_t* item_frame,
                                    const int32_t* choice, const double* pose, int B, int n_per, int r, int s_,
                                    uint64_t seed, int64_t item_offset, float* pts_out, float* box_out,
                                    float* init_box_out, hipStream_t st);
hipError_t launch_static_crop_labels(const double* points, const int64_t* offsets, const int32_t* choice, const double* pose,
                                     int B, int N, uint64_t seed, int64_t item_offset, const double* gt_planes,
                                     uint8_t* mask_label, hipStream_t s);
hipError_t launch_dynamic_item_labels(const double* points, const int64_t* frame_offsets, const int64_t* track_first,
                                      const int32_t* item_track, const int32_t* item_frame, const int32_t* choice,
                                      const double* pose, int B, int n_per, int r, uint64_t seed, int64_t item_offset,
                                      const double* xform, const double* planes, const uint8_t* valid, uint8_t* mask_label,
                                      hipStream_t st);
size_t crop_workspace_bytes(int64_t K_total, int64_t max_points_per_frame);
hipError_t launch_crop_count(const float* points, const int64_t* point_offsets, const double* planes,
                             const float* spheres, const int64_t* box_offsets, int F, int64_t K_total, int64_t max_points_per_frame,
                             int64_t* counts, int32_t* cc, hipStream_t s);
hipError_t launch_crop_fill(const float* points, const int64_t* point_offsets, const double* planes,
                            const float* spheres, const int64_t* box_offsets, int F, int64_t K_total,
                            int64_t max_points_per_frame, const double* pose, const int64_t* counts,
                            const int64_t* box_start, const int32_t* cc, double* out_points, int32_t* out_index,
                            int64_t out_capacity, hipStream_t s);
hipError_t launch_crop_starts(const int64_t* counts, const int64_t* order, int64_t K, int64_t* box_start, int64_t* out_offsets,
                              int64_t out_capacity, hipStream_t s);
int64_t box_iou_pairwise_blocks(int64_t n, int64_t m);
int64_t box_iou_paired_blocks(int64_t n);
hipError_t launch_box_iou_pairwise(const void* a, int64_t n, const void* b, int64_t m, int boxes_f64, float* iou_bev,
                                   float* iou_3d, hipStream_t s);
hipError_t launch_box_iou_paired(const void* a, const void* b, int64_t n, int boxes_f64, float* iou_bev, float* iou_3d,
                                 hipStream_t s);
int64_t box_estimation_metrics_chunks(int64_t N);
hipError_t launch_box_estimation_metrics(const dal3_box_metric_args* a, hipStream_t s);
size_t track_workspace_bytes(int64_t S, int64_t K, int64_t capacity);
size_t track_match_workspace_bytes(int64_t K);
hipError_t launch_track(const dal3_track_args* a, hipStream_t s);
hipError_t launch_track_match(const dal3_track_match_args* a, hipStream_t s);
size_t group_workspace_bytes(int64_t E, int64_t T);
size_t motion_classify_workspace_bytes(int64_t T);
hipError_t launch_group_by_key(const dal3_group_args* a, hipStream_t s);
hipError_t launch_track_features(const dal3_track_feature_args* a, hipStream_t s);
hipError_t launch_gt_table(const dal3_gt_table_args* a, hipStream_t s);
hipError_t launch_motion_classify(const dal3_motion_classify_args* a, hipStream_t s);
size_t score_workspace_bytes(int64_t S);
hipError_t launch_score_tracks(const dal3_score_args* a, hipStream_t s);
hipError_t launch_best_gt_iou(const dal3_best_gt_args* a, hipStream_t s);
size_t nms_workspace_bytes(int64_t K, int boxes_f64);
hipError_t launch_nms(const dal3_nms_args* a, hipStream_t s);
size_t center_decode_workspace_bytes(int64_t B, int64_t H, int64_t W);
hipError_t launch_center_decode(const dal3_center_decode_args* a, hipStream_t s);
hipError_t launch_center_decode_flip4(const dal3_center_decode_flip4_args* a, hipStream_t s);
hipError_t launch_flip4_points(const float* points, int64_t N, int C, const int64_t* offsets, int64_t B, float* out,
                               int64_t* out_offsets, int64_t max_workgroups, hipStream_t s);
// ... 227 lines not shown
```

3dal_pytorch_amd/csrc/dal3_misc.hip:

```cpp
#include "dal3_device.h"
#include "dal3_kernels.h"

#define BN_EPS 1e-5f

__device__ __forceinline__ float bn_scale(const dal3_layer& L, int row) {
    return L.bn_weight ? L.bn_weight[row] / sqrtf(L.bn_var[row] + BN_EPS) : 1.0f;
}

__device__ __forceinline__ float folded_w(const dal3_layer& L, int row, int col, int col_off, int n_cols) {
    if (row >= L.c_out || col >= n_cols) return 0.0f;
    return L.weight[(int64_t)row * L.c_in + col_off + col] * bn_scale(L, row);
}

__global__ void pack_weight_kernel(dal3_layer L, int mode, int col_off, int n_cols, int mt_n, int kt_n,
                                   float* __restrict__ out, int64_t total, int grp_blocks, int64_t grp_a0,
                                   int64_t grp_a1, int64_t grp_stride) {
    const int64_t i = (int64_t)blockIdx.x * blockDim.x + threadIdx.x;
    if (i >= total) return;
    if (mode == PACK_ROWMAJOR) {
        const int row = (int)(i / n_cols), col = (int)(i % n_cols);
        out[i] = folded_w(L, row, col, col_off, n_cols);
    } else if (mode == PACK_FIRST) {
        const int lane = (int)(i & 63);
        const int s = (int)((i >> 6) % kt_n), mt = (int)((i >> 6) / kt_n);
        out[i] = folded_w(L, 32 * mt + (lane & 31), 2 * s + (lane >> 5), col_off, n_cols);
    } else {
        const int e = (int)(i & 3), lane = (int)((i >> 2) & 63), q = (int)((i >> 8) & 3);
        const int blk = (int)(i >> 10);
        const int mt = mode == PACK_FRAG_MT_MAJOR ? blk / kt_n : blk % mt_n;
        const int kt = mode == PACK_FRAG_MT_MAJOR ? blk % kt_n : blk / mt_n;
        int64_t o = i;
        if (grp_blocks > 0) {
            const int g = blk / grp_blocks;
            o = (g == 0 ? grp_a0 : grp_a1 + (int64_t)(g - 1) * grp_stride) + (int64_t)(blk % grp_blocks) * 1024 + (i & 1023);
        }
        out[o] = folded_w(L, 32 * mt + (lane & 31), 32 * kt + tile_chan(4 * q + e, lane >> 5), col_off, n_cols);
    }
}

__global__ void pack_weight_lp_kernel(dal3_layer L, int dtype, int kt_major, int col_off, int n_cols, int mt_n, int kt_n,
                                      uint16_t* __restrict__ out, int64_t total, int grp_blocks, int64_t grp_a0,
                                      int64_t grp_a1, int64_t grp_stride) {
    const int64_t i = (int64_t)blockIdx.x * blockDim.x + threadIdx.x;
    if (i >= total) return;
    const int j = (int)(i & 7), lane = (int)((i >> 3) & 63), s = (int)((i >> 9) & 1);
    const int blk = (int)(i >> 10);
    const int mt = kt_major ? blk % mt_n : blk / kt_n;
    const int kt = kt_major ? blk / mt_n : blk % kt_n;
    const float v = folded_w(L, 32 * mt + (lane & 31), 32 * kt + 16 * s + 8 * (j >> 2) + 4 * (lane >> 5) + (j & 3), col_off,
                             n_cols);
    uint16_t bits;
    if (dtype == DAL3_BF16) {
        const __bf16 h = (__bf16)v;
        bits = __builtin_bit_cast(uint16_t, h);
    } else {
        const _Float16 h = (_Float16)v;
        bits = __builtin_bit_cast(uint16_t, h);
    }
    int64_t o = i;
    if (grp_blocks > 0) {
        const int g = blk / grp_blocks;
        o = (g == 0 ? grp_a0 : grp_a1 + (int64_t)(g - 1) * grp_stride) + (int64_t)(blk % grp_blocks) * 1024 + (i & 1023);
    }
    out[o] = bits;
}

__global__ void pack_weight_x3_kernel(dal3_layer L, int kt_major, int col_off, int n_cols, int mt_n, int kt_n,
                                      uint16_t* __restrict__ out, int64_t total, int grp_blocks, int64_t grp_a0,
                                      int64_t grp_a1, int64_t grp_stride, int64_t grp_last) {
    const int64_t i = (int64_t)blockIdx.x * blockDim.x + threadIdx.x;
    if (i >= total) return;
    const int j = (int)(i & 7), lane = (int)((i >> 3) & 63), half = (int)((i >> 9) & 1), s = (int)((i >> 10) & 1);
    const int blk = (int)(i >> 11);
    const int mt = kt_major ? blk % mt_n : blk / kt_n;
    const int kt = kt_major ? blk / mt_n : blk % kt_n;
    const float v = folded_w(L, 32 * mt + (lane & 31), 32 * kt + 16 * s + 8 * (j >> 2) + 4 * (lane >> 5) + (j & 3), col_off,
                             n_cols);
    const _Float16 hi = fabsf(v) < 65504.0f ? (_Float16)v : (_Float16)__builtin_nanf("");
    const _Float16 lo = (_Float16)(v - (float)hi);
    int64_t o = i;
    if (grp_blocks > 0) {
        const int g = blk / grp_blocks;
        const bool last = grp_last >= 0 && g == mt_n * kt_n / grp_blocks - 1;
        o = (last ? grp_last : g == 0 ? grp_a0 : grp_a1 + (int64_t)(g - 1) * grp_stride) + (int64_t)(blk % grp_blocks) * 2048 + (i & 2047);
// ... 16 lines not shown
    hipLaunchKernelGGL(pack_weight_lp_kernel, dim3((unsigned)((total + 255) / 256)), dim3(256), 0, s, L, dtype, kt_major,
                       col_off, n_cols, mt_n, kt_n, out, total, grp_blocks, grp_a0, grp_a1, grp_stride);
    return hipGetLastError();
}

__global__ void pack_bias_kernel(dal3_layer L, float* __restrict__ out, int padded) {
    const int i = blockIdx.x * blockDim.x + threadIdx.x;
    if (i >= padded) return;
    float v = 0.0f;
    if (i < L.c_out) {
        v = L.bias[i];
        if (L.bn_weight) v = (v - L.bn_mean[i]) * bn_scale(L, i) + L.bn_bias[i];
    }
    out[i] = v;
}

hipError_t launch_pack_weight(const dal3_layer& L, int mode, int col_off, int n_cols, int mt_n, int kt_n, float* out,
                              hipStream_t s, int grp_blocks, int64_t grp_a0, int64_t grp_a1, int64_t grp_stride) {
    int64_t total;
    if (mode == PACK_ROWMAJOR) total = (int64_t)L.c_out * n_cols;
    else if (mode == PACK_FIRST) total = (int64_t)mt_n * kt_n * 64;
    else total = (int64_t)mt_n * kt_n * 1024;
    hipLaunchKernelGGL(pack_weight_kernel, dim3((unsigned)((total + 255) / 256)), dim3(256), 0, s, L, mode, col_off,
                       n_cols, mt_n, kt_n, out, total, grp_blocks, grp_a0, grp_a1, grp_stride);
    return hipGetLastError();
}

__global__ void pack_enc_screen_kernel(dal3_layer L, float* __restrict__ pq, int32_t* __restrict__ flag) {
    const int c = blockIdx.x * blockDim.x + threadIdx.x;
    if (c >= 1024) return;
    double s2 = 0.0, s1 = 0.0;
    bool bad = false;
    for (int k = 0; k < 128; ++k) {
        const float v = folded_w(L, c, k, 0, 128);
        bad |= !(fabsf(v) < 65504.0f);
        s2 += (double)v * (double)v;
        s1 += fabs((double)v);
    }
    const double kappa = 1.02 * 0x1p-10 + 128.0 * 0x1p-23;
    pq[2 * c] = (float)((kappa * sqrt(s2) + 0x1p-24 * 11.3137085) * (1.0 + 1e-6));
    pq[2 * c + 1] = (float)((0x1p-24 * s1 + 0x1p-40) * (1.0 + 1e-6));
    if (bad) atomicOr(flag, 1);
}
hipError_t launch_pack_enc_screen(const dal3_layer& L, float* pq, int32_t* flag, hipStream_t s) {
    hipLaunchKernelGGL(pack_enc_screen_kernel, dim3(4), dim3(256), 0, s, L, pq, flag);
    return hipGetLastError();
}

__global__ void pack_head_screen_kernel(dal3_layer L, float* __restrict__ pq, int32_t* __restrict__ flag) {
    const int c = blockIdx.x * blockDim.x + threadIdx.x;
    if (c >= 512) return;
    double s2 = 0.0, s1 = 0.0;
    bool bad = false;
    for (int k = 0; k < 256; ++k) {
        const float v = folded_w(L, c, k, 0, 256);
        bad |= !(fabsf(v) < 65504.0f);
        s2 += (double)v * (double)v;
        s1 += fabs((double)v);
    }
    const double kappa = 1.02 * 0x1p-10 + 256.0 * 0x1p-23;
    pq[2 * c] = (float)((kappa * sqrt(s2) + 0x1p-24 * 16.0) * (1.0 + 1e-6));
    pq[2 * c + 1] = (float)((0x1p-24 * s1 + 0x1p-40) * (1.0 + 1e-6));
    if (bad) atomicOr(flag, 1);
}
hipError_t launch_pack_head_screen(const dal3_layer& L, float* pq, int32_t* flag, hipStream_t s) {
    hipLaunchKernelGGL(pack_head_screen_kernel, dim3(2), dim3(256), 0, s, L, pq, flag);
    return hipGetLastError();
}

__global__ void pack_dec_sparse_kernel(dal3_layer L, const float* __restrict__ db2, float* __restrict__ out,
                                       int32_t* __restrict__ flag) {
    const int i = blockIdx.x * blockDim.x + threadIdx.x;
    if (i >= 512 * 256) return;
    const int mt = i & 7, row = (i >> 3) & 31, k = i >> 8;
    const int c = k >> 5, r = (k & 31) >> 1, h = k & 1;
    const float v = folded_w(L, 32 * mt + row, 32 * c + tile_chan(r, h), 0, 512);
    out[i] = v;
    bool bad = (__float_as_uint(v) & 0x7F800000u) == 0x7F800000u;
    if (i < 256) bad |= __float_as_uint(db2[i]) == 0x80000000u;
    if (bad) atomicOr(flag, 1);
}
hipError_t launch_pack_dec_sparse(const dal3_layer& L, const float* db2, float* dw2c, int32_t* flag, hipStream_t s) {
    hipLaunchKernelGGL(pack_dec_sparse_kernel, dim3(512), dim3(256), 0, s, L, db2, dw2c, flag);
    return hipGetLastError();
}

__global__ void pack_dec_queue_kernel(dal3_layer L, int c_in, const float* __restrict__ bias, float* __restrict__ out,
                                      int32_t* __restrict__ flag) {
    const int i = blockIdx.x * blockDim.x + threadIdx.x;
    if (i >= c_in * 128) return;
    const int mt = i & 3, row = (i >> 2) & 31, k = i >> 7;
    const int kt = k >> 5, r = (k & 31) >> 1, h = k & 1;
    const float v = folded_w(L, 32 * mt + row, 32 * kt + tile_chan(r, h), 0, c_in);
    out[i] = v;
    bool bad = (__float_as_uint(v) & 0x7F800000u) == 0x7F800000u;
    if (i < 128) bad |= __float_as_uint(bias[i]) == 0x80000000u;
    if (bad) atomicOr(flag, 1);
}
hipError_t launch_pack_dec_queue(const dal3_layer& L, int c_in, const float* bias, float* wcopy, int32_t* flag, hipStream_t s) {
    hipLaunchKernelGGL(pack_dec_queue_kernel, dim3(c_in * 128 / 256), dim3(256), 0, s, L, c_in, bias, wcopy, flag);
    return hipGetLastError();
}

hipError_t launch_pack_bias(const dal3_layer& L, float* out, hipStream_t s) {
    const int padded = (L.c_out + 31) / 32 * 32;
    hipLaunchKernelGGL(pack_bias_kernel, dim3((padded + 255) / 256), dim3(256), 0, s, L, out, padded);
    return hipGetLastError();
}

__global__ __launch_bounds__(256) void fc_kernel(const float* __restrict__ W, const float* __restrict__ bias,
                                                 const float* __restrict__ x, int64_t xs, float* __restrict__ y,
                                                 int64_t ys, int B, int c_in, int c_out, int relu, int n_mt) {
    __shared__ float red[3][16][64];
    const int lane = threadIdx.x & 63;
    const int wave = threadIdx.x >> 6;
    const int h = lane >> 5;
    const int mt = blockIdx.x % n_mt, bt = blockIdx.x / n_mt;
    const int row = 32 * mt + (lane & 31);
    const int item = 32 * bt + (lane & 31);
    const bool row_ok = row < c_out, item_ok = item < B;
    const float* wp = W + (int64_t)(row_ok ? row : 0) * c_in + 4 * h;
    const float* xp = x + (int64_t)(item_ok ? item : 0) * xs + 4 * h;
    f32x16 acc;
#pragma unroll
    for (int r = 0; r < 16; ++r) {
        const int ch = 32 * mt + tile_chan(r, h);
        acc[r] = (wave == 0 && ch < c_out) ? bias[ch] : 0.0f;
    }
    const int chunk = ((c_in + 31) / 32) * 8;
    const int k_end = min(c_in, (wave + 1) * chunk);
    int k0 = wave * chunk;
    for (; k0 + 16 <= k_end; k0 += 16) {
        const f32x4 a0 = *reinterpret_cast<const f32x4*>(wp + k0);
        const f32x4 a1 = *reinterpret_cast<const f32x4*>(wp + k0 + 8);
        const f32x4 b0 = *reinterpret_cast<const f32x4*>(xp + k0);
        const f32x4 b1 = *reinterpret_cast<const f32x4*>(xp + k0 + 8);
#pragma unroll
        for (int e = 0; e < 4; ++e) acc = mfma32(a0[e], b0[e], acc);
#pragma unroll
        for (int e = 0; e < 4; ++e) acc = mfma32(a1[e], b1[e], acc);
    }
    for (; k0 < k_end; k0 += 8) {
        const f32x4 a = *reinterpret_cast<const f32x4*>(wp + k0);
        const f32x4 bv = *reinterpret_cast<const f32x4*>(xp + k0);
#pragma unroll
        for (int e = 0; e < 4; ++e) acc = mfma32(a[e], bv[e], acc);
    }
    if (wave > 0) {
#pragma unroll
        for (int r = 0; r < 16; ++r) red[wave - 1][r][lane] = acc[r];
    }
    __syncthreads();
    if (wave > 0 || !item_ok) return;
    float* yp = y + (int64_t)item * ys;
#pragma unroll
    for (int r = 0; r < 16; ++r) {
        const int ch = 32 * mt + tile_chan(r, h);
        const float v = ((acc[r] + red[0][r][lane]) + red[1][r][lane]) + red[2][r][lane];
        if (ch < c_out) yp[ch] = relu ? (v < 0.0f ? 0.0f : v) : v;
    }
}

hipError_t launch_fc(const float* W, const float* bias, const float* x, int64_t xs, float* y, int64_t ys, int B,
                     int c_in, int c_out, int relu, hipStream_t s) {
    if (c_in % 8 != 0 || xs % 4 != 0) return hipErrorInvalidValue;
    const int n_mt = (c_out + 31) / 32, n_bt = (B + 31) / 32;
// ... 863 lines not shown
```

3dal_pytorch_amd/csrc/dal3_pointmlp.hip:

```cpp
#include <stdlib.h>

#include "dal3_device.h"
#include "dal3_kernels.h"

#ifdef DAL3_STAMP
__device__ long long* g_stamps = nullptr;
extern "C" int dal3_debug_set_stamps(void* p) {
    return (int)hipMemcpyToSymbol(HIP_SYMBOL(g_stamps), &p, sizeof(p));
}
#define STAMP(k)                                                                                  \
    do {                                                                                          \
        __builtin_amdgcn_sched_barrier(0);                                                        \
        unsigned long long t_;                                                                    \
        asm volatile("s_memtime %0\n\ts_waitcnt lgkmcnt(0)" : "=s"(t_)::"memory");               \
        __builtin_amdgcn_sched_barrier(0);                                                        \
        if (lane == 0 && blockIdx.x < 2048) g_stamps[(blockIdx.x * DAL3_WG_WAVES + wave) * 8 + (k)] = t_; \
    } while (0)
#else
#define STAMP(k)
#endif

#ifndef DAL3_ENC_LDS_MAX
#define DAL3_ENC_LDS_MAX 1
#endif
template <int T>
__global__ __launch_bounds__(64 * DAL3_WG_WAVES) void ins_seg_encode_kernel(InsSegW w, BCN pts, int c_in, int n_pts,
                                                             int tiles_per_item, float* __restrict__ g) {
    const int lane = threadIdx.x & 63;
    const int wave = threadIdx.x >> 6;
    const int h = lane >> 5;
    const int64_t b = blockIdx.x / tiles_per_item;
    const int n0 = ((blockIdx.x % tiles_per_item) * DAL3_WG_WAVES + wave) * (32 * T);
    __shared__ float s_b5[1024];
    __shared__ int s_max[DAL3_ENC_LDS_MAX ? 1024 : 1];
    for (int i = threadIdx.x; i < 1024; i += 64 * DAL3_WG_WAVES) {
        s_b5[i] = w.b5[i];
        if (DAL3_ENC_LDS_MAX) s_max[i] = 0;
    }
    __syncthreads();
    if (n0 < n_pts) {
        WRing<DAL3_PF> ring;
        ring.init(w.enc_stream, lane);
        f32x16 bias = tile_from_channels(w.b2, h);
        float in[T][2];
        load_points<2, T>(pts, b, n0, n_pts, c_in, in, lane);
        f32x16 x1[T][2], x2[T][2], x3[T][2], x4[T][4];
        first_layer<2, 2, T>(w.w1, w.b1, in, x1, lane);
        mlp_layer_ring<2, 2, T>(ring, w.b2, w.b3, bias, x1, x2, lane);
        mlp_layer_ring<2, 2, T>(ring, w.b3, w.b4, bias, x2, x3, lane);
        mlp_layer_ring<2, 4, T>(ring, w.b4, w.b4, bias, x3, x4, lane);
        conv_max_layer<4, T>(ring, s_b5, x4, DAL3_ENC_LDS_MAX ? reinterpret_cast<float*>(s_max) : g + b * 1024, 32, lane);
    }
    if (DAL3_ENC_LDS_MAX) {
        __syncthreads();
        int* gi = reinterpret_cast<int*>(g + b * 1024);
        for (int c = threadIdx.x; c < 1024; c += 64 * DAL3_WG_WAVES) {
            const int v = s_max[c];
            if (v > 0) atomicMax(gi + c, v);
        }
    }
}

__device__ __forceinline__ uint64_t live_ballot(float v) {
    uint64_t bal;
    asm("v_cmp_ne_u32_e64 %0, 0, %1" : "=s"(bal) : "v"(v));
    return bal;
}
#ifndef DAL3_DEC_SPARSE
#define DAL3_DEC_SPARSE 1
#endif
#ifndef DAL3_DEC_NB
#define DAL3_DEC_NB 3
#endif
#ifndef DAL3_DEC_GROUP
#define DAL3_DEC_GROUP 4
#endif
static_assert(DAL3_DEC_GROUP == 1 || DAL3_DEC_GROUP == 2 || DAL3_DEC_GROUP == 4 || DAL3_DEC_GROUP == 8,
              "a group's rows fit the queue's 256, and the groups tile the 16 chunks");
static_assert(DAL3_PF == 8, "the compacted body's ring holds exactly one dconv1 chunk between two blocks");
#ifdef DAL3_DEC_COUNT
__device__ unsigned long long g_dec_count[12];
extern "C" int dal3_debug_dec_counts(unsigned long long* out, int reset) {
    hipError_t e = hipMemcpyFromSymbol(out, HIP_SYMBOL(g_dec_count), sizeof(g_dec_count));
    if (e == hipSuccess && reset) {
        unsigned long long z[12] = {};
        e = hipMemcpyToSymbol(HIP_SYMBOL(g_dec_count), z, sizeof(z));
    }
    return (int)e;
}
#endif
struct DecStep {
    f32x4 a0, a1;
    float b;
};

#ifndef DAL3_DEC_QNB
#define DAL3_DEC_QNB 4
#endif
#define DEC_Q_ZERO 256
#define DEC_Q_OVER 32
#define DEC_Q_LIST (256 + DEC_Q_OVER)
#define DEC_G_PEND ((DEC_Q_ZERO + 1) + DEC_Q_LIST / 32)
#define DEC_G_LIST ((DEC_G_PEND + 1) * 32)
#define DEC_Q_FLOATS (DEC_G_LIST + 2 * (1 + 256 + DEC_Q_OVER))
static_assert(DEC_Q_LIST % 32 == 0, "the leftover row starts where dconv3's list ends");
static_assert(4 * DAL3_DEC_QNB + 2 <= DEC_Q_OVER, "the loop reads list entries up to 2 (steps - 1 + 2 DAL3_DEC_QNB) + 1");
static_assert(4 * DAL3_DEC_NB + 2 <= DEC_Q_OVER, "dconv2's loop reads list entries up to 2 (steps - 1 + 2 DAL3_DEC_NB) + 1");
struct QStep {
    f32x4 a;
    float b;
};
template <int KT, int STAMP0>
__device__ __forceinline__ void dec_queue_layer(const f32x16 (&X)[KT], f32x16 (&Y)[4], const float* __restrict__ bvec,
                                                const float* __restrict__ wcopy, float* q, int lane, uint32_t& n_steps,
                                                uint32_t& n_live) {
    static_assert(KT % 2 == 0, "two k-tiles per 64-bit mask word");
    const uint32_t h = (uint32_t)lane >> 5, pt = (uint32_t)lane & 31u;
    uint32_t* kl = reinterpret_cast<uint32_t*>(q + (DEC_Q_ZERO + 1) * 32);
    const __amdgpu_buffer_rsrc_t wq = __builtin_amdgcn_make_buffer_rsrc(const_cast<float*>(wcopy), 0, KT * 32 * 512, 0x00020000);
    f32x16 acc[4];
#pragma unroll
    for (int mt = 0; mt < 4; ++mt) acc[mt] = tile_from_channels(bvec + 32 * mt, (int)h);
    __builtin_amdgcn_fence(__ATOMIC_ACQ_REL, "wavefront");
    __builtin_amdgcn_wave_barrier();
    uint32_t m[KT];
#pragma unroll
    for (int kt = 0; kt < KT; ++kt) {
        m[kt] = 0;
#pragma unroll
        for (int r = 0; r < 16; ++r) {
            const float v = X[kt][r];
            q[(32 * kt + 2 * r) * 32 + lane] = v;
            const uint64_t bal = live_ballot(v);
            uint32_t lo, hi;
            asm("s_min_u32 %1, %3, 1\n\ts_min_u32 %2, %4, 1\n\ts_lshl1_add_u32 %1, %2, %1\n\ts_lshl_b32 %1, %1, %5\n\ts_or_b32 %0, %0, %1"
                : "+s"(m[kt]), "=&s"(lo), "=&s"(hi)
                : "s"((uint32_t)bal), "s"((uint32_t)(bal >> 32)), "n"(2 * r)
                : "scc");
        }
    }
    q[DEC_Q_ZERO * 32 + pt] = 0.0f;
    uint32_t cnt = 0;
#pragma unroll
    for (int j = 0; j < KT / 2; ++j) {
        const uint32_t below = __builtin_amdgcn_mbcnt_hi(m[2 * j + 1], __builtin_amdgcn_mbcnt_lo(m[2 * j], 0u));
        const uint32_t word = h ? m[2 * j + 1] : m[2 * j];
        if ((word >> pt) & 1u) kl[cnt + below] = 64u * j + (uint32_t)lane;
        cnt += __builtin_popcount(m[2 * j]) + __builtin_popcount(m[2 * j + 1]);
    }
    if (lane < DEC_Q_OVER) kl[cnt + (uint32_t)lane] = DEC_Q_ZERO;
    __builtin_amdgcn_fence(__ATOMIC_ACQ_REL, "wavefront");
    __builtin_amdgcn_wave_barrier();
    const uint32_t steps = (cnt + 1u) >> 1;
    n_steps += steps, n_live += cnt;
#ifdef DAL3_STAMP
    const int wave = threadIdx.x >> 6;
    STAMP(STAMP0);
#endif
    auto mma = [&](const QStep& S) {
#pragma unroll
        for (int mt = 0; mt < 4; ++mt) acc[mt] = mfma32(S.a[mt], S.b, acc[mt]);
    };
    auto issue = [&](QStep& S, uint32_t k) {
        S.b = q[k * 32u + pt];
        S.a = __builtin_bit_cast(f32x4, __builtin_amdgcn_raw_buffer_load_b128(wq, k * 512u + pt * 16u, 0, 0));
    };
    const uint32_t* kp = kl + h;
    QStep S[DAL3_DEC_QNB];
    uint32_t K[DAL3_DEC_QNB];
#pragma unroll
    for (int u = 0; u < DAL3_DEC_QNB; ++u) K[u] = kp[2 * u];
#pragma unroll
    for (int u = 0; u < DAL3_DEC_QNB; ++u) {
        issue(S[u], K[u]);
        K[u] = kp[2 * (DAL3_DEC_QNB + u)];
    }
    uint32_t s = 0;
    for (; s + DAL3_DEC_QNB <= steps; s += DAL3_DEC_QNB) {
        kp += 2 * DAL3_DEC_QNB;
#pragma unroll
        for (int u = 0; u < DAL3_DEC_QNB; ++u) {
            mma(S[u]);
            issue(S[u], K[u]);
            K[u] = kp[2 * (DAL3_DEC_QNB + u)];
            DAL3_SCHED_FENCE();
        }
    }
#pragma unroll
    for (int u = 0; u + 1 < DAL3_DEC_QNB; ++u) {
        if (s + u < steps) mma(S[u]);
    }
#pragma unroll
    for (int mt = 0; mt < 4; ++mt) Y[mt] = relu16(acc[mt]);
}

template <int T, bool SP>
__device__ __forceinline__ void ins_seg_decode_tile(const InsSegW& w, const BCN& pts, int c_in, int n_pts, int64_t b, int n0,
                                                    const float* __restrict__ gb, float* __restrict__ logits,
                                                    uint8_t* __restrict__ mask, float* __restrict__ slab, int lane, int wave) {
    const int h = lane >> 5;
    STAMP(0);
    WRing<DAL3_PF> ring;
    ring.init(w.dec_stream, lane);
    f32x16 bias = tile_from_channels(w.b2, h);
    const bool crop_bad = bits_nonfinite(gb[0]);

    const int pt = lane & 31;
    __amdgpu_buffer_rsrc_t wc = ring.rsrc;
    constexpr int G = DAL3_DEC_GROUP;
    constexpr int TRIP = SP && G > 2 ? G : 2;
    uint32_t m[TRIP] = {};
    uint32_t pend = 0;
    typedef uint32_t u32x2 __attribute__((ext_vector_type(2)));
    u32x2 pend_e = {0u, DEC_Q_ZERO * 32u};
    u32x2* kl = reinterpret_cast<u32x2*>(slab + DEC_G_LIST);
    if constexpr (SP) {
        wc = __builtin_amdgcn_make_buffer_rsrc(const_cast<float*>(w.dw2c), 0, 512 * 1024, 0x00020000);
        slab[DEC_Q_ZERO * 32 + pt] = 0.0f;
    }
#ifdef DAL3_DEC_COUNT
    uint32_t n_dense = 0, n_comp = 0, n_steps = 0, n_live = 0;
#endif

    f32x16 x2[T][2];
    {
        float in[T][2];
        load_points<2, T>(pts, b, n0, n_pts, c_in, in, lane);
        f32x16 x1[T][2];
        first_layer<2, 2, T>(w.w1, w.b1, in, x1, lane);
        mlp_layer_ring<2, 2, T>(ring, w.b2, gb, bias, x1, x2, lane);
    }

    f32x16 a2[T][8];
#pragma unroll
    for (int mt = 0; mt < 8; ++mt) {
        const f32x16 b2v = tile_from_channels(w.db2 + 32 * mt, h);
#pragma unroll
        for (int j = 0; j < T; ++j) a2[j][mt] = b2v;
    }
    STAMP(1);
    f32x16 tA[T], tB[T];
    auto dconv2_part = [&](const f32x16 (&t)[T]) {
#pragma unroll
        for (int i = 0; i < 32; ++i) {
            ring_batch_wait<DAL3_PF>(ring, i);
            const f32x4 a = ring.slot[i % DAL3_PF];
            ring.slot[i % DAL3_PF] = ring.fetch();
#ifdef DAL3_ABLATE_WINDOW
            ring.soff &= ~0x2000u;
#endif
#pragma unroll
            for (int e = 0; e < 4; ++e) {
#pragma unroll
                for (int j = 0; j < T; ++j) a2[j][i / 4] = mfma32(a[e], t[j][4 * (i % 4) + e], a2[j][i / 4]);
            }
            DAL3_SCHED_FENCE();
        }
    };
    auto compact_mma = [&](const DecStep& S) {
#pragma unroll
        for (int mt = 0; mt < 8; ++mt) a2[0][mt] = mfma32(mt < 4 ? S.a0[mt & 3] : S.a1[mt & 3], S.b, a2[0][mt]);
    };
    auto compact_issue = [&](DecStep& S, u32x2 e) {
        const uint32_t voff = e[0] + (uint32_t)pt * 32u;
        S.b = slab[e[1] + (uint32_t)pt];
        S.a0 = __builtin_bit_cast(f32x4, __builtin_amdgcn_raw_buffer_load_b128(wc, voff, 0, 0));
        S.a1 = __builtin_bit_cast(f32x4, __builtin_amdgcn_raw_buffer_load_b128(wc, voff + 16u, 0, 0));
    };
    auto dconv2_group = [&](int c0, const uint32_t* mg) {
        constexpr int NG = G;
        __builtin_amdgcn_fence(__ATOMIC_ACQ_REL, "wavefront");
        __builtin_amdgcn_wave_barrier();
        kl[0] = pend_e;
        uint32_t total = pend;
#pragma unroll
        for (int j = 0; j < (NG + 1) / 2; ++j) {
            const uint32_t w0 = mg[2 * j], w1 = 2 * j + 1 < NG ? mg[2 * j + 1] : 0u;
            const uint32_t below = __builtin_amdgcn_mbcnt_hi(w1, __builtin_amdgcn_mbcnt_lo(w0, 0u));
            const uint32_t word = h ? w1 : w0;
            if ((word >> pt) & 1u) {
                u32x2 e;
                e[0] = (32u * (uint32_t)(c0 + 2 * j) + (uint32_t)lane) * 1024u;
                e[1] = (64u * j + (uint32_t)lane) * 32u;
                kl[total + below] = e;
            }
            total += __builtin_popcount(w0) + __builtin_popcount(w1);
        }
        if (lane < DEC_Q_OVER) {
            u32x2 e;
            e[0] = 0u, e[1] = DEC_Q_ZERO * 32u;
            kl[total + (uint32_t)lane] = e;
        }
        __builtin_amdgcn_fence(__ATOMIC_ACQ_REL, "wavefront");
        __builtin_amdgcn_wave_barrier();
        const uint32_t steps = total >> 1;
        const u32x2* kp = kl + h;
        DecStep S[DAL3_DEC_NB];
        u32x2 K[DAL3_DEC_NB];
#pragma unroll
        for (int u = 0; u < DAL3_DEC_NB; ++u) K[u] = kp[2 * u];
#pragma unroll
        for (int u = 0; u < DAL3_DEC_NB; ++u) {
            compact_issue(S[u], K[u]);
            K[u] = kp[2 * (DAL3_DEC_NB + u)];
        }
        if (total & 1u) {
            pend_e = kl[total - 1u];
            const float v = slab[pend_e[1] + (uint32_t)pt];
            __builtin_amdgcn_fence(__ATOMIC_ACQ_REL, "wavefront");
            slab[DEC_G_PEND * 32 + pt] = v;
            __builtin_amdgcn_fence(__ATOMIC_ACQ_REL, "wavefront");
            __builtin_amdgcn_wave_barrier();
            pend_e[1] = DEC_G_PEND * 32u;
        }
        pend = total & 1u;
        uint32_t s = 0;
        for (; s + DAL3_DEC_NB <= steps; s += DAL3_DEC_NB) {
            kp += 2 * DAL3_DEC_NB;
#pragma unroll
            for (int u = 0; u < DAL3_DEC_NB; ++u) {
                compact_mma(S[u]);
                compact_issue(S[u], K[u]);
                K[u] = kp[2 * (DAL3_DEC_NB + u)];
                DAL3_SCHED_FENCE();
            }
        }
#pragma unroll
        for (int u = 0; u + 1 < DAL3_DEC_NB; ++u) {
            if (s + u < steps) compact_mma(S[u]);
        }
#ifdef DAL3_DEC_COUNT
        n_comp += NG, n_steps += steps;
#pragma unroll
        for (int j = 0; j < NG; ++j) n_live += __builtin_popcount(mg[j]);
#endif
    };
    auto dconv2_chunk = [&](const f32x16 (&t)[T], int c, int u) {
        if constexpr (SP) {
            if ((u + 1) % G == 0) dconv2_group(c + 1 - G, m + (u + 1 - G));
        } else {
#ifdef DAL3_DEC_COUNT
            ++n_dense, n_live += 32;
#endif
            dconv2_part(t);
        }
    };
    auto relu_note = [&](f32x16& t, int i, int u) {
        t[2 * i] = relu1(t[2 * i]);
        t[2 * i + 1] = relu1(t[2 * i + 1]);
        if constexpr (SP) {
            if (i == 0) m[u] = 0;
#pragma unroll
            for (int r = 2 * i; r < 2 * i + 2; ++r) {
                const float v = t[r];
                slab[(32 * (u % G) + 2 * r) * 32 + lane] = v;
                const uint64_t bal = live_ballot(v);
                uint32_t lo, hi;
                asm("s_min_u32 %1, %3, 1\n\ts_min_u32 %2, %4, 1\n\ts_lshl1_add_u32 %1, %2, %1\n\ts_lshl_b32 %1, %1, %5\n\ts_or_b32 %0, %0, %1"
                    : "+s"(m[u]), "=&s"(lo), "=&s"(hi)
                    : "s"((uint32_t)bal), "s"((uint32_t)(bal >> 32)), "n"(2 * r)
                    : "scc");
            }
        }
    };
    auto skip_dconv2 = [&]() {
        if constexpr (SP) ring.soff += 32 * 1024;
    };
#pragma unroll
    for (int j = 0; j < T; ++j) tA[j] = bias;
    mma_block_ring<2, T>(ring, x2, tA, [&](int i) {
        if (i == 0) bias = tile_from_channels(gb + 32, h);
    });
    for (int c0 = 0; c0 < 16; c0 += TRIP) {
#pragma unroll
        for (int u = 0; u < TRIP; u += 2) {
            const int c = c0 + u;
#pragma unroll
            for (int j = 0; j < T; ++j) tB[j] = bias;
            skip_dconv2();
            mma_block_ring<2, T>(ring, x2, tB, [&](int i) {
                if (i == 0) bias = tile_from_channels(gb + 32 * ((c + 2) & 15), h);
#pragma unroll
                for (int j = 0; j < T; ++j) relu_note(tA[j], i, u);
            });
            dconv2_chunk(tA, c, u);
#pragma unroll
            for (int j = 0; j < T; ++j) tA[j] = bias;
            skip_dconv2();
            mma_block_ring<2, T>(ring, x2, tA, [&](int i) {
                if (i == 0)
                    bias = c + 2 < 16 ? tile_from_channels(gb + 32 * ((c + 3) & 15), h) : tile_from_channels(w.db3, h);
#pragma unroll
                for (int j = 0; j < T; ++j) relu_note(tB[j], i, u + 1);
            });
            dconv2_chunk(tB, c + 1, u + 1);
        }
    }
    if constexpr (SP) {
        if (pend) {
            DecStep S;
            u32x2 e = pend_e;
            if (h) e[1] = DEC_Q_ZERO * 32u;
            compact_issue(S, e);
            compact_mma(S);
#ifdef DAL3_DEC_COUNT
            ++n_steps;
#endif
        }
    }
#ifdef DAL3_DEC_COUNT
    if (lane == 0) {
        atomicAdd(&g_dec_count[0], 1ull);
        atomicAdd(&g_dec_count[5], SP ? 1ull : 0ull);
        atomicAdd(&g_dec_count[1], (unsigned long long)n_dense);
        atomicAdd(&g_dec_count[2], (unsigned long long)n_comp);
        atomicAdd(&g_dec_count[3], (unsigned long long)n_steps);
        atomicAdd(&g_dec_count[4], (unsigned long long)n_live);
    }
#endif
    STAMP(2);
#pragma unroll
    for (int j = 0; j < T; ++j) {
#pragma unroll
        for (int mt = 0; mt < 8; ++mt) a2[j][mt] = relu16(a2[j][mt]);
    }

    f32x16 y3[T][4], y4[T][4];
    if constexpr (SP) {
        uint32_t q_steps3 = 0, q_live3 = 0, q_steps4 = 0, q_live4 = 0;
        dec_queue_layer<8, 5>(a2[0], y3[0], w.db3, w.dw3c, slab, lane, q_steps3, q_live3);
        STAMP(6);
        dec_queue_layer<4, 7>(y3[0], y4[0], w.db4, w.dw4c, slab, lane, q_steps4, q_live4);
#ifdef DAL3_DEC_COUNT
        if (lane == 0) {
            atomicAdd(&g_dec_count[6], (unsigned long long)q_steps3);
            atomicAdd(&g_dec_count[7], (unsigned long long)q_live3);
            atomicAdd(&g_dec_count[8], (unsigned long long)q_steps4);
            atomicAdd(&g_dec_count[9], (unsigned long long)q_live4);
        }
#endif
    } else {
        mlp_layer_ring<8, 4, T>(ring, w.db3, w.db4, bias, a2, y3, lane);
        mlp_layer_ring<4, 4, T>(ring, w.db4, w.db4, bias, y3, y4, lane);
    }

    STAMP(3);
    float l0[T], l1[T];
#pragma unroll
    for (int j = 0; j < T; ++j) l0[j] = l1[j] = 0.0f;
#pragma unroll
    for (int kt = 0; kt < 4; ++kt) {
#pragma unroll
        for (int q = 0; q < 4; ++q) {
            const f32x4 wa = *reinterpret_cast<const f32x4*>(w.dw5 + 32 * kt + 8 * q + 4 * h);
            const f32x4 wb = *reinterpret_cast<const f32x4*>(w.dw5 + 128 + 32 * kt + 8 * q + 4 * h);
#pragma unroll
            for (int e = 0; e < 4; ++e) {
#pragma unroll
                for (int j = 0; j < T; ++j) {
                    l0[j] = fmaf(wa[e], y4[j][kt][4 * q + e], l0[j]);
                    l1[j] = fmaf(wb[e], y4[j][kt][4 * q + e], l1[j]);
                }
            }
        }
    }
    const float bias0 = w.db5[0], bias1 = w.db5[1];
#pragma unroll
    for (int j = 0; j < T; ++j) {
        float s0 = l0[j] + __shfl_xor(l0[j], 32) + bias0;
        float s1 = l1[j] + __shfl_xor(l1[j], 32) + bias1;
        if (crop_bad) s0 = s1 = __int_as_float(DAL3_QNAN_BITS);
        const int n = n0 + 32 * j + (lane & 31);
        if (h == 0 && n < n_pts) {
            f32x2 o;
            o[0] = s0;
            o[1] = s1;
            *reinterpret_cast<f32x2*>(logits + (b * n_pts + n) * 2) = o;
            mask[b * n_pts + n] = (!crop_bad && s0 < s1) ? 1 : 0;
        }
    }
    STAMP(4);
}

#ifndef DAL3_DEC_MIN_DEAD
#define DAL3_DEC_MIN_DEAD 64
#endif
template <int T>
__global__ __launch_bounds__(64 * DAL3_WG_WAVES) void ins_seg_decode_kernel(InsSegW w, BCN pts, int c_in, int n_pts,
                                                             int tiles_per_item, const float* __restrict__ gbias,
                                                             float* __restrict__ logits, uint8_t* __restrict__ mask) {
    const int lane = threadIdx.x & 63;
    const int wave = threadIdx.x >> 6;
#ifndef DAL3_DEC_XCD
#define DAL3_DEC_XCD 1
#endif
    unsigned blk = blockIdx.x;
    if (DAL3_DEC_XCD) {
        const unsigned per = gridDim.x >> 3, rem = gridDim.x & 7u, x = blockIdx.x & 7u;
        blk = x * per + (x < rem ? x : rem) + (blockIdx.x >> 3);
    }
    const int64_t b = blk / tiles_per_item;
    const int n0 = ((blk % tiles_per_item) * DAL3_WG_WAVES + wave) * (32 * T);
    if (n0 >= n_pts) return;
    const float* gb = gbias + b * 512;
    constexpr bool SP = DAL3_DEC_SPARSE != 0 && T == 1;
    extern __shared__ __attribute__((aligned(16))) float s_slab[];
    if constexpr (SP) {
        const f32x4 g0 = reinterpret_cast<const f32x4*>(gb)[2 * lane], g1 = reinterpret_cast<const f32x4*>(gb)[2 * lane + 1];
        uint32_t neg = 0;
#pragma unroll
        for (int e = 0; e < 4; ++e)
            neg += __builtin_popcountll(__builtin_amdgcn_ballot_w64(__float_as_int(g0[e]) < 0)) +
                   __builtin_popcountll(__builtin_amdgcn_ballot_w64(__float_as_int(g1[e]) < 0));
        if (neg >= DAL3_DEC_MIN_DEAD && *w.dec_flag == 0) {
            ins_seg_decode_tile<T, true>(w, pts, c_in, n_pts, b, n0, gb, logits, mask, s_slab + wave * DEC_Q_FLOATS, lane, wave);
            return;
        }
    }
    asm volatile(".p2align 8");
    ins_seg_decode_tile<T, false>(w, pts, c_in, n_pts, b, n0, gb, logits, mask, s_slab, lane, wave);
}

template <int KS, int C1, int C2, int C3, int T>
__global__ __launch_bounds__(64 * DAL3_WG_WAVES) void point_head_kernel(PointHeadW w, BCN x, int c_in, int n_pts,
                                                         int tiles_per_item, float* __restrict__ feat,
                                                         const int32_t* __restrict__ distinct) {
    const int lane = threadIdx.x & 63;
    const int wave = threadIdx.x >> 6;
    const int h = lane >> 5;
    const int wg_waves = blockDim.x >> 6;
    const int n_items = gridDim.x / tiles_per_item;
    const int64_t b = blockIdx.x % n_items;
    const int n0 = ((blockIdx.x / n_items) * wg_waves + wave) * (32 * T);
    __shared__ float s_b4[512];
    for (int i = threadIdx.x; i < 512; i += blockDim.x) s_b4[i] = w.b4[i];
    __syncthreads();
    if (distinct) {
        const int d = distinct[b];
        n_pts = d <= 0 ? 1 : (d < n_pts ? d : n_pts);
    }
    if (n0 >= n_pts) return;

    WRing<DAL3_PF> ring;
    ring.init(w.stream, lane);
    f32x16 bias = tile_from_channels(w.b2, h);
    f32x16 x3[T][C3 / 32];
    {
        float in[T][KS];
        load_points<KS, T>(x, b, n0, n_pts, c_in, in, lane);
        f32x16 x1[T][C1 / 32], x2[T][C2 / 32];
        first_layer<KS, C1 / 32, T>(w.w1, w.b1, in, x1, lane);
        mlp_layer_ring<C1 / 32, C2 / 32, T>(ring, w.b2, w.b3, bias, x1, x2, lane);
        mlp_layer_ring<C2 / 32, C3 / 32, T>(ring, w.b3, w.b3, bias, x2, x3, lane);
    }
    conv_max_layer<C3 / 32, T>(ring, s_b4, x3, feat + b * 512, 16, lane);
}

#ifndef HEAD_RUN
#define HEAD_RUN 6
#endif
template <int KS, int C1, int C2, int C3>
__global__ __launch_bounds__(64) void point_head_pers_kernel(PointHeadW w, BCN x, int c_in, float* __restrict__ feat,
                                                             uint32_t* __restrict__ ctl, const u32x4* __restrict__ list) {
    constexpr int T = 1;
    const int lane = threadIdx.x & 63;
    const int h = lane >> 5;
    __shared__ float s_b4[512];
    __shared__ int s_run[512];
    for (int i = threadIdx.x; i < 512; i += 64) {
        s_b4[i] = w.b4[i];
        s_run[i] = 0;
    }
    __syncthreads();
    const uint32_t n_live = ctl[0];
    uint32_t run0 = n_live / (2u * gridDim.x);
    run0 = run0 < 1u ? 1u : (run0 > HEAD_RUN ? HEAD_RUN : run0);
    const uint32_t first_free = gridDim.x * run0;
    uint32_t cur = blockIdx.x * run0, run_end = cur + run0;
    if (cur >= n_live) return;

    constexpr uint32_t STREAM_BYTES =
        ((C2 / 32) * (C1 / 32) + (C3 / 32) * (C2 / 32) + 16 * (C3 / 32)) * 4u * 1024u;
    WRing<DAL3_PF, true> ring;
    ring.init(w.stream, lane, STREAM_BYTES);
    f32x16 bias = tile_from_channels(w.b2, h);
    u32x4 e = list[cur];
    float in[T][KS];
    load_points<KS, T>(x, (int64_t)e[0], (int)e[1] * 32, (int)e[2], c_in, in, lane);
    auto flush = [&](int64_t b) {
        int* gi = reinterpret_cast<int*>(feat + b * 512);
#pragma unroll
        for (int c = lane; c < 512; c += 64) {
            const int v = s_run[c];
            if (v > 0) atomicMax(gi + c, v);
            s_run[c] = 0;
        }
    };
    for (;;) {
// ... 24 lines not shown
            e = list[nclamp];
            mlp_layer_ring<C2 / 32, C3 / 32, T>(ring, w.b3, w.b2, bias, x2, x3, lane);
            load_points<KS, T>(x, (int64_t)e[0], (int)e[1] * 32, (int)e[2], c_in, in_n, lane);
        }
        conv_max_layer<C3 / 32, T>(ring, s_b4, x3, reinterpret_cast<float*>(s_run), 16, lane);
        const bool more = ncur < n_live;
        if (!more || (int64_t)e[0] != b) flush(b);
        if (!more) break;
        cur = ncur;
        run_end = nend;
#pragma unroll
        for (int k = 0; k < KS; ++k) in[0][k] = in_n[0][k];
    }
}

__global__ __launch_bounds__(256) void generic_layer_kernel(const f32x4* __restrict__ wf, const float* __restrict__ w1,
                                                            const float* __restrict__ bias, int kt_n, int ks_n, int mt_n,
                                                            int relu, BCN x, int c_in, int n_pts, int tiles_per_item,
                                                            float* __restrict__ y) {
    const int lane = threadIdx.x & 63;
    const int wave = threadIdx.x >> 6;
    const int h = lane >> 5;
    const int64_t b = blockIdx.x / tiles_per_item;
    const int n0 = ((blockIdx.x % tiles_per_item) * 4 + wave) * 32;
    if (n0 >= n_pts) return;
    int n = n0 + (lane & 31);
    const bool valid = n < n_pts;
    n = valid ? n : n_pts - 1;
    const float* p = x.data + b * x.sb + (int64_t)n * x.sn;
    const int c_out = 32 * mt_n;
    for (int mt = 0; mt < mt_n; ++mt) {
        f32x16 acc = tile_from_channels(bias + 32 * mt, h);
        if (ks_n > 0) {
            for (int s = 0; s < ks_n; ++s) {
                const int c = 2 * s + h;
                const float bv = c < c_in ? p[c * x.sc] : 0.0f;
                acc = mfma32(w1[(mt * ks_n + s) * 64 + lane], bv, acc);
            }
        } else {
            for (int kt = 0; kt < kt_n; ++kt) {
                for (int q = 0; q < 4; ++q) {
                    const f32x4 a = wf[((mt * kt_n + kt) * 4 + q) * 64 + lane];
#pragma unroll
                    for (int e = 0; e < 4; ++e) {
                        const int c = 32 * kt + 8 * q + 4 * h + e;
                        acc = mfma32(a[e], p[c * x.sc], acc);
                    }
                }
            }
        }
        if (relu) acc = relu16(acc);
        if (valid) {
#pragma unroll
            for (int q = 0; q < 4; ++q) {
                f32x4 o;
                o[0] = acc[4 * q + 0];
                o[1] = acc[4 * q + 1];
                o[2] = acc[4 * q + 2];
                o[3] = acc[4 * q + 3];
                *reinterpret_cast<f32x4*>(y + (b * n_pts + n) * c_out + 32 * mt + 8 * q + 4 * h) = o;
            }
        }
    }
}

static inline int tiles_per_item(int n_pts, int T) {
    return (n_pts + 32 * DAL3_WG_WAVES * T - 1) / (32 * DAL3_WG_WAVES * T);
}

#ifndef DAL3_LAT_MAX_TILES
#define DAL3_LAT_MAX_TILES 512
#endif
#ifndef DAL3_LAT_MAX_TILES_ENC
#define DAL3_LAT_MAX_TILES_ENC DAL3_LAT_MAX_TILES
#endif
#ifndef DAL3_LAT_MAX_TILES_DEC
#define DAL3_LAT_MAX_TILES_DEC DAL3_LAT_MAX_TILES
#endif
#ifndef DAL3_LAT_MAX_TILES_HEAD
#define DAL3_LAT_MAX_TILES_HEAD DAL3_LAT_MAX_TILES
#endif
bool lat_use(int64_t tiles, int flags, int64_t max_tiles) { return !(flags & DAL3_BCN_NO_SMALL_JOB_KERNELS) && tiles <= max_tiles; }

hipError_t launch_ins_seg_encode(const InsSegW& w, BCN pts, int c_in, int B, int N, float* g, hipStream_t s) {
    if (lat_use((int64_t)B * ((N + 31) / 32), pts.flags, DAL3_LAT_MAX_TILES_ENC)) return launch_ins_seg_encode_lat(w, pts, c_in, B, N, g, s);
    constexpr int T = DAL3_ENC_T;
    if (T > 1 && (int64_t)B * N <= 1024 * 64) {
        const int tpi1 = tiles_per_item(N, 1);
        hipLaunchKernelGGL(ins_seg_encode_kernel<1>, dim3((unsigned)((int64_t)B * tpi1)), dim3(64 * DAL3_WG_WAVES), 0, s, w, pts, c_in, N, tpi1, g);
        return hipGetLastError();
    }
    if (DAL3_ENC_SCREEN) return launch_ins_seg_encode_screen(w, pts, c_in, B, N, g, s);
    const int tpi = tiles_per_item(N, T);
    hipLaunchKernelGGL(ins_seg_encode_kernel<T>, dim3((unsigned)((int64_t)B * tpi)), dim3(64 * DAL3_WG_WAVES), 0, s, w, pts, c_in, N, tpi, g);
    return hipGetLastError();
}

hipError_t launch_ins_seg_decode(const InsSegW& w, BCN pts, int c_in, int B, int N, const float* gbias,
                                 float* logits, uint8_t* mask, hipStream_t s) {
    if (lat_use((int64_t)B * ((N + 31) / 32), pts.flags, DAL3_LAT_MAX_TILES_DEC)) return launch_ins_seg_decode_lat(w, pts, c_in, B, N, gbias, logits, mask, s);
    constexpr int T = DAL3_DEC_T;
    const int tpi = tiles_per_item(N, T);
    constexpr size_t lds = DAL3_DEC_SPARSE != 0 && T == 1 ? (size_t)DAL3_WG_WAVES * DEC_Q_FLOATS * sizeof(float) : 0;
    if (lds) {
        const hipError_t e = hipFuncSetAttribute(reinterpret_cast<const void*>(ins_seg_decode_kernel<T>),
                                                 hipFuncAttributeMaxDynamicSharedMemorySize, (int)lds);
        if (e != hipSuccess) return e;
    }
    hipLaunchKernelGGL(ins_seg_decode_kernel<T>, dim3((unsigned)((int64_t)B * tpi)), dim3(64 * DAL3_WG_WAVES), lds, s, w, pts, c_in, N, tpi,
                       gbias, logits, mask);
    return hipGetLastError();
}

size_t point_head_worklist_bytes(int B, int M) { return 256 + (size_t)B * ((M + 31) / 32) * sizeof(u32x4); }

static int head_slots() {
    int dev = 0, v = 0;
    if (hipGetDevice(&dev) != hipSuccess || hipDeviceGetAttribute(&v, hipDeviceAttributeMultiprocessorCount, dev) != hipSuccess || v <= 0)
        v = 256;
    return 4 * v;
}

hipError_t launch_point_head(int head_kind, const PointHeadW& w, BCN x, int c_in, int B, int M, float* feat,
                             const int32_t* distinct, hipStream_t s, void* worklist, size_t worklist_bytes) {
    constexpr int T = DAL3_HEAD_T;
    const int tpi = (M + 32 * T - 1) / (32 * T);
    const bool lat = lat_use((int64_t)B * ((M + 31) / 32), x.flags, DAL3_LAT_MAX_TILES_HEAD);
    const bool pers = !lat && worklist && worklist_bytes >= point_head_worklist_bytes(B, M) && !(x.flags & DAL3_BCN_NO_WORKLIST) && T == 1;
    const bool screen = DAL3_HEAD_SCREEN && pers && (head_kind == 1 || head_kind == 2) && w.w4row &&
                        (int64_t)B * tpi >= DAL3_HEAD_SCR_MIN_TILES && tpi > 1;
    hipError_t e0 = launch_nonfinite_rows(x, B, M, c_in, feat, 512, s, distinct, pers ? worklist : nullptr,
                                          screen ? DAL3_HEAD_SCR_STRIDE : 0);
    if (e0 != hipSuccess) return e0;
    if (lat) return launch_point_head_lat(head_kind, w, x, c_in, B, M, feat, distinct, s);
    if (pers) {
        uint32_t* ctl = static_cast<uint32_t*>(worklist);
        u32x4* list = reinterpret_cast<u32x4*>(static_cast<char*>(worklist) + 256);
        const int64_t slots = head_slots();
        const int64_t seed_tpi = (tpi + DAL3_HEAD_SCR_STRIDE - 1) / DAL3_HEAD_SCR_STRIDE;
        const int64_t tiles = screen ? (int64_t)B * seed_tpi : (int64_t)B * tpi;
        const dim3 grid((unsigned)(tiles < slots ? tiles : slots)), block(64);
        switch (head_kind) {
            case 1:
                hipLaunchKernelGGL((point_head_pers_kernel<2, 128, 128, 256>), grid, block, 0, s, w, x, c_in, feat, ctl, list);
                break;
            case 2:
                hipLaunchKernelGGL((point_head_pers_kernel<2, 64, 128, 256>), grid, block, 0, s, w, x, c_in, feat, ctl, list);
                break;
            case 3:
                hipLaunchKernelGGL((point_head_pers_kernel<4, 64, 64, 128>), grid, block, 0, s, w, x, c_in, feat, ctl, list);
                break;
            default:
                return hipErrorInvalidValue;
        }
        hipError_t e1 = hipGetLastError();
        if (e1 != hipSuccess || !screen) return e1;
        return launch_point_head_screen(head_kind, w, x, c_in, feat, ctl + 2, list + (size_t)B * seed_tpi,
                                        (int64_t)B * (tpi - seed_tpi), slots, s);
    }
    const dim3 grid((unsigned)((int64_t)B * tpi)), block(64);
    switch (head_kind) {
        case 1:
            hipLaunchKernelGGL((point_head_kernel<2, 128, 128, 256, T>), grid, block, 0, s, w, x, c_in, M, tpi, feat, distinct);
            break;
        case 2:
            hipLaunchKernelGGL((point_head_kernel<2, 64, 128, 256, T>), grid, block, 0, s, w, x, c_in, M, tpi, feat, distinct);
            break;
        case 3:
            hipLaunchKernelGGL((point_head_kernel<4, 64, 64, 128, T>), grid, block, 0, s, w, x, c_in, M, tpi, feat, distinct);
            break;
        default:
            return hipErrorInvalidValue;
    }
    return hipGetLastError();
}

hipError_t launch_generic_layer(const f32x4* wf, const float* w1, const float* bias, int kt_n, int ks_n, int mt_n,
                                int relu, BCN x, int c_in, int B, int N, float* y, hipStream_t s) {
    const int tpi = (N + 127) / 128;
    hipLaunchKernelGGL(generic_layer_kernel, dim3((unsigned)((int64_t)B * tpi)), dim3(256), 0, s, wf, w1, bias, kt_n,
                       ks_n, mt_n, relu, x, c_in, N, tpi, y);
    return hipGetLastError();
}
```

3dal_pytorch_amd/csrc/dal3_screen.h:

```cpp
#pragma once
#include "dal3_device.h"


__device__ __forceinline__ uint32_t scr_push_hit(uint32_t hb, float acc, float k) {
    return __builtin_amdgcn_alignbit(hb, __float_as_uint(k - acc), 31);
}

template <int T>
__host__ __device__ constexpr uint32_t scr_tile_mask(int j) {
    uint32_t m = 0;
    for (int s = j; s < 16 * T; s += T) m |= 1u << (16 * T - 1 - s);
    return m;
}

template <int T>
struct ScreenHits {
    uint32_t n[T];
    uint32_t nz;
    __device__ __forceinline__ void init() {
#pragma unroll
        for (int j = 0; j < T; ++j) n[j] = 0;
        nz = 0;
    }
    __device__ __forceinline__ void park_block(uint32_t* park, int mt, uint32_t hb, int lane) {
        hb &= (uint32_t)((1ull << (16 * T)) - 1ull);
        park[mt * 64 + lane] = hb;
#pragma unroll
        for (int j = 0; j < T; ++j) n[j] += (uint32_t)__builtin_popcount(hb & scr_tile_mask<T>(j));
        nz = (nz << 1) | (hb < 1u ? hb : 1u);
    }
};

template <int T, int NBLK, int CAP>
__device__ __forceinline__ bool scr_build_lists(const uint32_t* park, uint32_t* list, ScreenHits<T> hits, uint32_t (&cnt)[T], int lane) {
    static_assert(16 * T <= 32 && NBLK <= 32, "one hit word per block, one block bit per word");
    const int h = lane >> 5;
    uint32_t pos[T];
    bool overflow = false;
#pragma unroll
    for (int j = 0; j < T; ++j) {
        uint32_t incl = hits.n[j];
#pragma unroll
        for (int d = 1; d < 64; d <<= 1) {
            const uint32_t up = (uint32_t)__shfl_up((int)incl, d);
            incl += lane >= d ? up : 0u;
        }
        pos[j] = incl - hits.n[j];
        cnt[j] = (uint32_t)__builtin_amdgcn_readlane((int)incl, 63);
        overflow |= cnt[j] > (uint32_t)CAP;
    }
    if (overflow) return true;
    uint32_t nz = hits.nz, w = 0;
    int mt = 0;
    for (;;) {
        if (w == 0) {
            if (nz == 0) break;
            mt = NBLK - 1 - __builtin_ctz(nz);
            nz &= nz - 1;
            w = park[mt * 64 + lane];
        }
        const int s = 16 * T - 1 - __builtin_ctz(w);
        w &= w - 1;
        const int j = s % T, r = s / T;
        const uint32_t e = ((uint32_t)(32 * mt + (lane & 31)) << 8) | (uint32_t)tile_chan(r, h);
        uint32_t at = 0;
#pragma unroll
        for (int jj = 0; jj < T; ++jj) {
            at = j == jj ? (uint32_t)(jj * CAP) + pos[jj] : at;
            pos[jj] += j == jj ? 1u : 0u;
        }
        list[at] = e;
    }
    return false;
}

template <int SW, int NS, int DEPTH, bool EARLY, typename A0, typename Fin>
__device__ __forceinline__ void scr_recompute(const float* __restrict__ wrow, int ldw, const uint32_t* list, uint32_t cnt,
                                              const float* xw, int xld, uint32_t* stage, int lane, A0&& a0, Fin&& fin) {
    static_assert(SW == 16 || SW == 32, "a slice is 4 or 8 lanes of 16 bytes per candidate");
    static_assert(DEPTH >= 1 && NS % DEPTH == 0, "slices in flight: slice q lives in registers q % DEPTH, round after round");
    constexpr int LPC = SW / 4, LD = SW + 4;
    const int sub = lane / LPC, piece = lane % LPC;
    u32x4 wq[DEPTH][LPC];
    uint32_t off[LPC], noff[EARLY ? LPC : 1];
    auto served = [&](uint32_t base, uint32_t (&o)[LPC]) {
#pragma unroll
        for (int t = 0; t < LPC; ++t) {
            const uint32_t idx = base + (64 / LPC) * t + sub;
            o[t] = (list[idx < cnt ? idx : 0u] >> 8) * (uint32_t)(ldw * 4) + (uint32_t)(16 * piece);
// ... 58 lines not shown
```

include/dal3.h:

```cpp
#ifndef DAL3_H
#define DAL3_H

#include <stddef.h>
#include <stdint.h>

#ifdef __cplusplus
extern "C" {
#endif

typedef void* dal3_stream;

#define DAL3_VERSION 170

enum {
    DAL3_OK = 0,
    DAL3_EINVAL = -1,
    DAL3_EWORKSPACE = -2,
    DAL3_EHIP = -3
};

#define DAL3_MAX_ITEMS 16777216
#define DAL3_MAX_POINTS_PER_ITEM 16777216
#define DAL3_MAX_TILES 2147483647

enum { DAL3_F32 = 0, DAL3_BF16 = 1, DAL3_F16 = 2,
       DAL3_F16X3 = 3 };

enum {
    DAL3_HEAD_INS_SEG = 0,
    DAL3_HEAD_STATIC_BOX_EST = 1,
    DAL3_HEAD_POINT_EMB = 2,
    DAL3_HEAD_BOX_EMB = 3,
    DAL3_HEAD_DYNAMIC_BOX_EST = 4
};

enum {
    DAL3_SAMPLER_DEVICE = 0,
    DAL3_SAMPLER_CHOICE = 1
};

typedef struct {
    const float* weight;
    const float* bias;
    const float* bn_weight;
    const float* bn_bias;
    const float* bn_mean;
    const float* bn_var;
    int32_t c_in;
    int32_t c_out;
} dal3_layer;

int dal3_version(void);
const char* dal3_last_error(void);
const float* dal3_mean_size(void);

int dal3_pack_weights(int head_kind, const dal3_layer* layers, int n_layers, int dtype,
                      void* packed_dev, size_t* bytes_inout, dal3_stream stream);

typedef struct {
    const float* data;
    int64_t stride_b, stride_c, stride_n;
    int32_t dtype;
    int32_t flags;
} dal3_bcn;

enum { DAL3_BCN_NO_SMALL_JOB_KERNELS = 1, DAL3_BCN_NO_WORKLIST = 2, DAL3_BCN_NO_LDS_SAMPLER = 4 };

size_t dal3_ins_seg_workspace_bytes(int B);
int dal3_ins_seg_forward(const void* packed, int dtype, int c_in, dal3_bcn pts, int B, int N,
                         float* logits, uint8_t* mask, float* global_feat_out,
                         void* workspace, size_t workspace_bytes, dal3_stream stream);

int dal3_ins_seg_encode(const void* packed, int dtype, int c_in, dal3_bcn pts, int B, int N, float* global_feat,
                        dal3_stream stream);
int dal3_ins_seg_global_bias(const void* packed, int dtype, const float* global_feat, int B, float* gbias,
                             dal3_stream stream);
int dal3_ins_seg_decode(const void* packed, int dtype, int c_in, dal3_bcn pts, int B, int N, const float* gbias,
                        float* logits, uint8_t* mask, dal3_stream stream);

size_t dal3_gather_workspace_bytes(int B, int N);
int dal3_segment_counts(const uint8_t* mask, int B, int N, int32_t* counts, dal3_stream stream);
int dal3_mask_compact_sample(const uint8_t* mask, dal3_bcn pts, int B, int N, int C, int M,
                             int sampler, const int32_t* choice, uint64_t seed, int64_t item_offset,
                             int32_t* counts, int32_t* obj_idx, float* obj_pts,
                             void* workspace, size_t workspace_bytes, dal3_stream stream);

int dal3_mask_compact_sample_step(const uint8_t* mask, dal3_bcn pts, int B, int N, int C, int M, uint64_t seed,
                                  const int64_t* step, int64_t item_offset, int32_t* counts, int32_t* obj_idx,
                                  float* obj_pts, void* workspace, size_t workspace_bytes, dal3_stream stream);

size_t dal3_point_head_workspace_bytes(int B);
int dal3_point_head_forward(int head_kind, const void* packed, int dtype, dal3_bcn x, int B, int M,
                            float* out, int64_t out_stride,
                            void* workspace, size_t workspace_bytes, dal3_stream stream);

size_t dal3_point_head_pool_workspace_bytes(int B, int M);
int dal3_point_head_pool(int head_kind, const void* packed, int dtype, dal3_bcn x, int B, int M,
                         const int32_t* n_distinct, float* feat, void* workspace, size_t workspace_bytes,
                         dal3_stream stream);
int dal3_point_head_screen_min_tiles(void);
int dal3_point_head_screen_stride(void);

int dal3_dynamic_box_est_forward(const void* packed, const float* embedding, int B, float* box_pred,
                                 void* workspace, size_t workspace_bytes, dal3_stream stream);

int dal3_decode_boxes(float* box_pred, int B,
                      const float* center_add, int64_t center_add_stride, int center_inplace,
                      const float* boxes_center_add, int64_t boxes_center_add_stride,
                      const float* yaw_base, int64_t yaw_stride,
                      float* heading_residuals, float* size_residuals, float* center, float* boxes7,
                      dal3_stream stream);

int dal3_recenter_rotz(const float* obj_pts, int B, int M, const float* init_box7,
                       const float* box_one7, const float* bbox_gt7, float* obj_pts_two,
                       int64_t* heading_class_label, float* heading_residual_label,
                       dal3_stream stream);

int dal3_maxpool_n(const float* x, int64_t rows, int64_t n, float* out, dal3_stream stream);
int dal3_maxpool_n_dtype(const void* x, int dtype, int64_t rows, int64_t n, void* out, dal3_stream stream);

int dal3_static_crop_prep(const double* points, const int64_t* offsets, const int32_t* choice,
                          const double* pose, const double* box, int B, int N, uint64_t seed,
                          int64_t item_offset, float* pts_out, float* init_box_out, dal3_stream stream);

int dal3_dynamic_item_prep(const double* points, const int64_t* frame_offsets, const double* boxes,
                           const int64_t* track_first, const int32_t* item_track, const int32_t* item_frame,
                           const int32_t* choice, const double* pose, int B, int n_per, int r, int s,
                           uint64_t seed, int64_t item_offset, float* pts_out, float* box_out,
                           float* init_box_out, dal3_stream stream);

int dal3_writeback_boxes(const double* final_boxes, const int32_t* final_idx, const double* pose_best,
                         const double* pose_inv, const double* track_box, float* det, const int64_t* det_start,
                         const int32_t* det_count, const uint8_t* active, int P, int64_t n_det, int32_t* match,
                         int32_t* owner, dal3_stream stream);

int dal3_static_crop_labels(const double* points, const int64_t* offsets, const int32_t* choice, const double* pose,
                            int B, int N, uint64_t seed, int64_t item_offset, const double* gt_planes,
                            uint8_t* mask_label, dal3_stream stream);
int dal3_dynamic_item_labels(const double* points, const int64_t* frame_offsets, const int64_t* track_first,
                             const int32_t* item_track, const int32_t* item_frame, const int32_t* choice,
                             const double* pose, int B, int n_per, int r, uint64_t seed, int64_t item_offset,
                             const double* xform, const double* planes, const uint8_t* valid, uint8_t* mask_label,
                             dal3_stream stream);

int dal3_points_in_boxes(const void* points, int points_f64, int64_t P, int64_t stride, const double* planes, int K,
                         int f32_math, uint8_t* inside, dal3_stream stream);

int dal3_box_iou_pairwise(const void* a, int64_t n, const void* b, int64_t m, int boxes_f64, float* iou_bev,
                          float* iou_3d, dal3_stream stream);
int dal3_box_iou_paired(const void* a, const void* b, int64_t n, int boxes_f64, float* iou_bev, float* iou_3d,
                        dal3_stream stream);
// ... 962 lines not shown
```

Baseline: 233,700 object-crops/s.

## Plan per-item dead decoder channels from encoder bounds to prune decode work

Adds a pruning sweep inside the instance-segmentation encoder's second screen pass that computes per-channel upper bounds on the decoder's first-layer pre-activations using fp16 MFMA plus error bounds. A new plan kernel then combines these with the global bias to list, per item, which decoder channels can be nonzero, and the sparse decode tile iterates only over those compacted channels. The aim is to cut decoder conv1/conv2 work, at the cost of an extra encoder sweep, a memset, a plan kernel, larger workspace and LDS, and reliance on a conservative bound for exactness.

```diff
diff --git a/3dal_pytorch_amd/_hip.py b/3dal_pytorch_amd/_hip.py
--- a/3dal_pytorch_amd/_hip.py
+++ b/3dal_pytorch_amd/_hip.py
@@ -352,6 +352,7 @@
     "dal3_mean_size": (C.POINTER(C.c_float), []),
     "dal3_pack_weights": (_i, [_i, C.POINTER(Layer), _i, _i, vp, C.POINTER(_sz), vp]),
     "dal3_ins_seg_workspace_bytes": (_sz, [_i]),
+    "dal3_ins_seg_plan_layout": (_i, [_i, C.POINTER(_sz), C.POINTER(_i)]),
     "dal3_ins_seg_forward": (_i, [vp, _i, _i, BCN, _i, _i, vp, vp, vp, vp, _sz, vp]),
     "dal3_ins_seg_encode": (_i, [vp, _i, _i, BCN, _i, _i, vp, vp]),
     "dal3_ins_seg_global_bias": (_i, [vp, _i, vp, _i, vp, vp]),
@@ -578,6 +579,7 @@
 
 STORAGE = {torch.float32: F32, torch.bfloat16: BF16, torch.float16: F16}
 BCN_NO_SMALL_JOB_KERNELS, BCN_NO_WORKLIST, BCN_NO_LDS_SAMPLER = 1, 2, 4
+BCN_NO_DEC_PLAN = 16
 DISPATCH_FLAGS = 0
 
 
diff --git a/3dal_pytorch_amd/csrc/dal3_api.hip b/3dal_pytorch_amd/csrc/dal3_api.hip
--- a/3dal_pytorch_amd/csrc/dal3_api.hip
+++ b/3dal_pytorch_amd/csrc/dal3_api.hip
@@ -65,6 +65,11 @@
     w.dw2c = c.take((size_t)512 * 256);
     w.dw3c = c.take((size_t)256 * 128);
     w.dw4c = c.take((size_t)128 * 128);
+    w.dw1c = c.take((size_t)(DEC_NULL_K + 1) * 64);
+    w.w1h = c.take4((size_t)16 * 2 * 2 * 256);
+    w.prn_pq = c.take(2 * 512);
+    w.dec_ident = reinterpret_cast<const uint32_t*>(c.take(DEC_PLAN_LD));
+    w.prn_flag = reinterpret_cast<const int32_t*>(c.take(64));
     w.dec_flag = reinterpret_cast<const int32_t*>(c.take(64));
     return w;
 }
@@ -418,6 +423,9 @@
         HIP_TRY(launch_pack_dec_sparse(L[6], w.db2, mut(w.dw2c), reinterpret_cast<int32_t*>(const_cast<int32_t*>(w.dec_flag)), s));
         HIP_TRY(launch_pack_dec_queue(L[7], 256, w.db3, mut(w.dw3c), reinterpret_cast<int32_t*>(const_cast<int32_t*>(w.dec_flag)), s));
         HIP_TRY(launch_pack_dec_queue(L[8], 128, w.db4, mut(w.dw4c), reinterpret_cast<int32_t*>(const_cast<int32_t*>(w.dec_flag)), s));
+        HIP_TRY(launch_pack_weight_lp(L[5], DAL3_F16, 0, 0, 64, 16, 2, reinterpret_cast<uint16_t*>(mut(w.w1h)), s));
+        HIP_TRY(launch_pack_dec_prune(L[5], mut(w.dw1c), mut(w.prn_pq), const_cast<uint32_t*>(w.dec_ident),
+                                      const_cast<int32_t*>(w.prn_flag), s));
         return 0;
     }
     if (head_kind == DAL3_HEAD_DYNAMIC_BOX_EST) {
@@ -486,7 +494,7 @@
     if (t.dtype != DAL3_F32 && t.dtype != DAL3_BF16 && t.dtype != DAL3_F16)
         return fail(DAL3_EINVAL, "%s: storage dtype %d is none of DAL3_F32 / DAL3_BF16 / DAL3_F16", what, t.dtype);
     if (t.dtype != DAL3_F32 && (reinterpret_cast<uintptr_t>(t.data) & 1)) return fail(DAL3_EINVAL, "%s: 16-bit data must be 2-byte aligned", what);
-    if (t.flags & ~(DAL3_BCN_NO_SMALL_JOB_KERNELS | DAL3_BCN_NO_WORKLIST | DAL3_BCN_NO_LDS_SAMPLER)) return fail(DAL3_EINVAL, "%s: unknown bits in flags (%d)", what, t.flags);
+    if (t.flags & ~(DAL3_BCN_NO_SMALL_JOB_KERNELS | DAL3_BCN_NO_WORKLIST | DAL3_BCN_NO_LDS_SAMPLER | DAL3_BCN_NO_DEC_PLAN)) return fail(DAL3_EINVAL, "%s: unknown bits in flags (%d)", what, t.flags);
     return 0;
 }
 
@@ -501,17 +509,32 @@
     return 0;
 }
 
-struct InsSegWs { float* g; float* gb; };
+struct InsSegWs { float* g; float* gb; uint32_t* prune; uint32_t* plan_k; float* plan_gbc; int32_t* plan_nch; };
 static InsSegWs carve_ins_seg(Carver& c, int B) {
     InsSegWs w;
     w.g = c.take<float>((size_t)B * 1024);
     w.gb = c.take<float>((size_t)B * 512);
+    w.prune = c.take<uint32_t>((size_t)B * 513);
+    w.plan_k = c.take<uint32_t>((size_t)B * DEC_PLAN_LD);
+    w.plan_gbc = c.take<float>((size_t)B * 512);
+    w.plan_nch = c.take<int32_t>((size_t)B);
     return w;
 }
 extern "C" size_t dal3_ins_seg_workspace_bytes(int B) {
     Carver c(nullptr, 0);
     carve_ins_seg(c, B);
     return c.off;
+}
+
+extern "C" int dal3_ins_seg_plan_layout(int B, size_t off[4], int* min_dead) {
+    if (B <= 0 || !off) return fail(DAL3_EINVAL, "ins_seg_plan_layout: bad argument");
+    char* const origin = reinterpret_cast<char*>(uintptr_t(4096));
+    Carver c(origin, ~size_t(0));
+    const InsSegWs w = carve_ins_seg(c, B);
+    off[0] = reinterpret_cast<char*>(w.prune) - origin, off[1] = reinterpret_cast<char*>(w.plan_k) - origin;
+    off[2] = reinterpret_cast<char*>(w.plan_gbc) - origin, off[3] = reinterpret_cast<char*>(w.plan_nch) - origin;
+    if (min_dead) *min_dead = DAL3_DEC_MIN_DEAD;
+    return 0;
 }
 
 static int check_dtype(int dtype) {
@@ -531,9 +554,13 @@
     HIP_TRY(launch_nonfinite_rows(x, B, N, c_in, ws.g, 1024, s));
     if (dtype == DAL3_F32) {
         const InsSegW w = ins_seg_view(static_cast<const float*>(packed), c_in);
-        HIP_TRY(launch_ins_seg_encode(w, x, c_in, B, N, ws.g, s));
+        const bool plan = dec_plan_route(x.flags, B, N);
+        if (plan) HIP_TRY(hipMemsetAsync(ws.prune, 0, (size_t)B * 513 * sizeof(uint32_t), s));
+        HIP_TRY(launch_ins_seg_encode(w, x, c_in, B, N, ws.g, s, plan ? ws.prune : nullptr));
         HIP_TRY(launch_fc(w.dw1g, w.db1, ws.g, 1024, ws.gb, 512, B, 1024, 512, 0, s));
-        HIP_TRY(launch_ins_seg_decode(w, x, c_in, B, N, ws.gb, logits, mask, s));
+        if (plan) HIP_TRY(launch_dec_plan(w, ws.gb, ws.prune, B, ws.plan_k, ws.plan_gbc, ws.plan_nch, s));
+        HIP_TRY(launch_ins_seg_decode(w, x, c_in, B, N, ws.gb, logits, mask, s,
+                                      plan ? DecPlan{ws.plan_k, ws.plan_gbc, ws.plan_nch} : DecPlan{nullptr, nullptr, nullptr}));
     } else if (dtype == DAL3_F16X3) {
         const InsSegX3W w = ins_seg_x3_view(packed);
         HIP_TRY(launch_ins_seg_encode_x3(w, x, c_in, B, N, ws.g, s));
diff --git a/3dal_pytorch_amd/csrc/dal3_enc_screen.hip b/3dal_pytorch_amd/csrc/dal3_enc_screen.hip
--- a/3dal_pytorch_amd/csrc/dal3_enc_screen.hip
+++ b/3dal_pytorch_amd/csrc/dal3_enc_screen.hip
@@ -35,9 +35,70 @@
 #define SCR_COUNT(k, v)
 #endif
 
+template <int T>
+__device__ __forceinline__ void dec_prune_sweep(const InsSegW& w, const f32x16 (&x2)[T][2], uint32_t* s_u, int* s_x, int lane) {
+    int xm = 0;
+    float x2max = 0.0f;
+#pragma unroll
+    for (int j = 0; j < T; ++j) {
+        float ss = 0.0f;
+#pragma unroll
+        for (int kt = 0; kt < 2; ++kt) {
+#pragma unroll
+            for (int r = 0; r < 16; ++r) {
+                const int v = __float_as_int(x2[j][kt][r]);
+                xm = v > xm ? v : xm;
+                ss = fmaf(x2[j][kt][r], x2[j][kt][r], ss);
+            }
+        }
+        ss += __shfl_xor(ss, 32);
+        x2max = __builtin_fmaxf(x2max, ss);
+    }
+#pragma unroll
+    for (int d = 16; d >= 1; d >>= 1) x2max = __builtin_fmaxf(x2max, __shfl_xor(x2max, d));
+    const bool over = *w.prn_flag != 0 || __builtin_amdgcn_ballot_w64(xm > SCR_XMAX_BITS) != 0;
+    const float X = sqrtf(x2max) * (1.0f + 0x1p-16f);
+    if (lane == 0) atomicMax(s_x, over ? 0x7F800000 : __float_as_int(X));
+    if (over) return;
+    ActTile<FP16> xh[T][2];
+#pragma unroll
+    for (int j = 0; j < T; ++j) {
+#pragma unroll
+        for (int kt = 0; kt < 2; ++kt) xh[j][kt] = pack_relu<FP16>(x2[j][kt]);
+    }
+    WRing<4> r16;
+    r16.init(w.w1h, lane);
+    f32x16 acc[2][T];
+    auto fold = [&](const f32x16 (&a)[T], int mt) {
+        float m = a[0][0];
+#pragma unroll
+        for (int j = 0; j < T; ++j) {
+#pragma unroll
+            for (int r = (j == 0 ? 1 : 0); r < 16; ++r) m = __builtin_fmaxf(m, a[j][r]);
+        }
+        m = __builtin_fmaxf(m, __shfl_xor(m, 32));
+        if (lane < 32) atomicMax(&s_u[32 * mt + lane], prune_key(__float_as_uint(m)));
+    };
+#pragma unroll
+    for (int mt = 0; mt < 16; ++mt) {
+#pragma unroll
+        for (int j = 0; j < T; ++j) acc[mt & 1][j] = f32x16{};
+#pragma unroll
+        for (int i = 0; i < 4; ++i) {
+            const f16x8_t a = __builtin_bit_cast(f16x8_t, r16.slot[i]);
+            r16.slot[i] = r16.fetch();
+#pragma unroll
+            for (int j = 0; j < T; ++j) acc[mt & 1][j] = FP16::mfma(xh[j][i >> 1].k[i & 1], a, acc[mt & 1][j]);
+        }
+        if (mt > 0) fold(acc[(mt - 1) & 1], mt - 1);
+    }
+    fold(acc[1], 15);
+}
+
 template <int PASS, int T>
 __global__ __launch_bounds__(64 * DAL3_WG_WAVES) void ins_seg_encode_screen_kernel(InsSegW w, BCN pts, int c_in, int n_pts,
-                                                                                  int tiles_per_item, float* __restrict__ g) {
+                                                                                  int tiles_per_item, float* __restrict__ g,
+                                                                                  uint32_t* __restrict__ prune) {
     const int lane = threadIdx.x & 63;
     const int wave = threadIdx.x >> 6;
     const int h = lane >> 5;
@@ -50,8 +111,10 @@
     __shared__ __attribute__((aligned(16))) float s_x[PASS == 1 ? DAL3_WG_WAVES * 32 * SCR_XLD : 4];
     __shared__ uint32_t s_list[PASS == 1 ? DAL3_WG_WAVES * T * SCR_CAP : 1];
     __shared__ __attribute__((aligned(16))) uint32_t s_stage[PASS == 1 ? DAL3_WG_WAVES * 64 * SCR_STAGE_LD : 4];
+    __shared__ uint32_t s_u[PASS == 1 ? 512 : 1];
+    __shared__ int s_xn[1];
     int* gi = reinterpret_cast<int*>(g + b * 1024);
-    static_assert(20 * 1024 + DAL3_WG_WAVES * (32 * SCR_XLD * 4 + T * SCR_CAP * 4 + 64 * SCR_STAGE_LD * 4) <= 160 * 1024,
+    static_assert(22 * 1024 + 64 + DAL3_WG_WAVES * (32 * SCR_XLD * 4 + T * SCR_CAP * 4 + 64 * SCR_STAGE_LD * 4) <= 160 * 1024,
                   "pass B's LDS exceeds a CU's 160 KiB: lower SCR_CAP, DAL3_WG_WAVES or DAL3_ENC_T");
     static_assert(32 * 64 <= 64 * SCR_STAGE_LD, "a wave's stage holds the hit words of conv5's 32 blocks");
     if (PASS == 0 && *w.scr_flag != 0) return;
@@ -60,7 +123,9 @@
         s_max[i] = 0;
         s_pq[i] = reinterpret_cast<const f32x2*>(w.scr_pq)[i];
         if (PASS == 1) s_g[i] = __int_as_float(__hip_atomic_load(gi + i, __ATOMIC_RELAXED, __HIP_MEMORY_SCOPE_AGENT));
-    }
+        if (PASS == 1 && i < 512) s_u[i] = 0;
+    }
+    if (threadIdx.x == 0) s_xn[0] = 0;
     __syncthreads();
     if (n0 < n_pts) {
         WRing<DAL3_PF> ring;
@@ -71,6 +136,7 @@
         f32x16 x1[T][2], x2[T][2], x3[T][2], x4[T][4];
         first_layer<2, 2, T>(w.w1, w.b1, in, x1, lane);
         mlp_layer_ring<2, 2, T>(ring, w.b2, w.b3, bias, x1, x2, lane);
+        if (PASS == 1 && prune) dec_prune_sweep<T>(w, x2, s_u, s_xn, lane);
         mlp_layer_ring<2, 2, T>(ring, w.b3, w.b4, bias, x2, x3, lane);
         mlp_layer_ring<2, 4, T>(ring, w.b4, w.b4, bias, x3, x4, lane);
         SCR_COUNT(0, 1);
@@ -240,17 +306,25 @@
         const int v = s_max[c];
         if (v > 0) atomicMax(gi + c, v);
     }
+    if (PASS == 1 && prune) {
+        uint32_t* pu = prune + b * 513;
+        for (int c = threadIdx.x; c < 512; c += 64 * DAL3_WG_WAVES) {
+            const uint32_t v = s_u[c];
+            if (v > 0) atomicMax(pu + c, v);
+        }
+        if (threadIdx.x == 0 && s_xn[0] > 0) atomicMax(reinterpret_cast<int*>(pu + 512), s_xn[0]);
+    }
 }
 
-hipError_t launch_ins_seg_encode_screen(const InsSegW& w, BCN pts, int c_in, int B, int N, float* g, hipStream_t s) {
+hipError_t launch_ins_seg_encode_screen(const InsSegW& w, BCN pts, int c_in, int B, int N, float* g, hipStream_t s, uint32_t* prune) {
     constexpr int T = DAL3_ENC_T;
     const int tpi = (N + 32 * DAL3_WG_WAVES * T - 1) / (32 * DAL3_WG_WAVES * T);
     const int slots = (N + 32 * T - 1) / (32 * T);
     const int tpi_a = ((slots + DAL3_SCR_A_STRIDE - 1) / DAL3_SCR_A_STRIDE + DAL3_WG_WAVES - 1) / DAL3_WG_WAVES;
     const dim3 grid_a((unsigned)((int64_t)B * tpi_a)), grid((unsigned)((int64_t)B * tpi)), block(64 * DAL3_WG_WAVES);
-    hipLaunchKernelGGL((ins_seg_encode_screen_kernel<0, T>), grid_a, block, 0, s, w, pts, c_in, N, tpi_a, g);
+    hipLaunchKernelGGL((ins_seg_encode_screen_kernel<0, T>), grid_a, block, 0, s, w, pts, c_in, N, tpi_a, g, nullptr);
     hipError_t e = hipGetLastError();
     if (e != hipSuccess) return e;
-    hipLaunchKernelGGL((ins_seg_encode_screen_kernel<1, T>), grid, block, 0, s, w, pts, c_in, N, tpi, g);
+    hipLaunchKernelGGL((ins_seg_encode_screen_kernel<1, T>), grid, block, 0, s, w, pts, c_in, N, tpi, g, prune);
     return hipGetLastError();
 }
diff --git a/3dal_pytorch_amd/csrc/dal3_kernels.h b/3dal_pytorch_amd/csrc/dal3_kernels.h
--- a/3dal_pytorch_amd/csrc/dal3_kernels.h
+++ b/3dal_pytorch_amd/csrc/dal3_kernels.h
@@ -61,6 +61,24 @@
     const float* dw3c;
     const float* dw4c;
     const int32_t* dec_flag;
+    const float* dw1c;
+    const f32x4* w1h;
+    const float* prn_pq;
+    const uint32_t* dec_ident;
+    const int32_t* prn_flag;
+};
+#ifndef DAL3_DEC_MIN_DEAD
+#define DAL3_DEC_MIN_DEAD 64
+#endif
+#ifndef DAL3_DEC_PLAN_ROUND
+#define DAL3_DEC_PLAN_ROUND 2
+#endif
+#define DEC_PLAN_LD 640
+#define DEC_NULL_K 512
+struct DecPlan {
+    const uint32_t* k;
+    const float* gbc;
+    const int32_t* nch;
 };
 enum {
     ENC_W2 = 0, ENC_W3 = 16, ENC_W4 = 32, ENC_W5 = 64, ENC_FRAGS = 64 + 512,
@@ -176,13 +194,17 @@
 FcW fc_head_view(const float* base);
 void point_head_dims(int head_kind, int* c_in, int* ks, int c[4], int* n_fc, int fc_in[3], int fc_out[3]);
 
-hipError_t launch_ins_seg_encode(const InsSegW& w, BCN pts, int c_in, int B, int N, float* g, hipStream_t s);
-hipError_t launch_ins_seg_encode_screen(const InsSegW& w, BCN pts, int c_in, int B, int N, float* g, hipStream_t s);
+hipError_t launch_ins_seg_encode(const InsSegW& w, BCN pts, int c_in, int B, int N, float* g, hipStream_t s, uint32_t* prune = nullptr);
+hipError_t launch_ins_seg_encode_screen(const InsSegW& w, BCN pts, int c_in, int B, int N, float* g, hipStream_t s, uint32_t* prune);
+bool dec_plan_route(int flags, int B, int N);
+hipError_t launch_pack_dec_prune(const dal3_layer& L, float* dw1c, float* pq, uint32_t* ident, int32_t* flag, hipStream_t s);
+hipError_t launch_dec_plan(const InsSegW& w, const float* gb, const uint32_t* prune, int B, uint32_t* plan_k, float* plan_gbc,
+                           int32_t* plan_nch, hipStream_t s);
 hipError_t launch_pack_enc_screen(const dal3_layer& L, float* pq, int32_t* flag, hipStream_t s);
 hipError_t launch_pack_dec_sparse(const dal3_layer& L, const float* db2, float* dw2c, int32_t* flag, hipStream_t s);
 hipError_t launch_pack_dec_queue(const dal3_layer& L, int c_in, const float* bias, float* wcopy, int32_t* flag, hipStream_t s);
 hipError_t launch_ins_seg_decode(const InsSegW& w, BCN pts, int c_in, int B, int N, const float* gbias,
-                                 float* logits, uint8_t* mask, hipStream_t s);
+                                 float* logits, uint8_t* mask, hipStream_t s, DecPlan plan = DecPlan{nullptr, nullptr, nullptr});
 size_t point_head_worklist_bytes(int B, int M);
 hipError_t launch_point_head(int head_kind, const PointHeadW& w, BCN x, int c_in, int B, int M, float* feat,
                              const int32_t* distinct, hipStream_t s, void* worklist = nullptr, size_t worklist_bytes = 0);
diff --git a/3dal_pytorch_amd/csrc/dal3_misc.hip b/3dal_pytorch_amd/csrc/dal3_misc.hip
--- a/3dal_pytorch_amd/csrc/dal3_misc.hip
+++ b/3dal_pytorch_amd/csrc/dal3_misc.hip
@@ -1,5 +1,6 @@
 #include "dal3_device.h"
 #include "dal3_kernels.h"
+#include "dal3_screen.h"
 
 #define BN_EPS 1e-5f
 
@@ -182,6 +183,80 @@
 }
 hipError_t launch_pack_dec_sparse(const dal3_layer& L, const float* db2, float* dw2c, int32_t* flag, hipStream_t s) {
     hipLaunchKernelGGL(pack_dec_sparse_kernel, dim3(512), dim3(256), 0, s, L, db2, dw2c, flag);
+    return hipGetLastError();
+}
+
+__global__ void pack_dec_prune_kernel(dal3_layer L, float* __restrict__ dw1c, float* __restrict__ pq, uint32_t* __restrict__ ident,
+                                      int32_t* __restrict__ flag) {
+    const int i = blockIdx.x * blockDim.x + threadIdx.x;
+    if (i < (DEC_NULL_K + 1) * 64) {
+        const int k = i >> 6, hh = (i >> 5) & 1, f = i & 31;
+        const int ch = 32 * (k >> 5) + tile_chan((k & 31) >> 1, k & 1);
+        dw1c[i] = k < DEC_NULL_K ? folded_w(L, ch, 32 * (f >> 4) + tile_chan(f & 15, hh), 0, 64) : 0.0f;
+    }
+    if (i < DEC_PLAN_LD) ident[i] = i < DEC_NULL_K ? (uint32_t)i : (uint32_t)DEC_NULL_K;
+    if (i >= 512) return;
+    double s2 = 0.0, s1 = 0.0;
+    bool bad = false;
+    for (int k = 0; k < 64; ++k) {
+        const float v = folded_w(L, i, k, 0, 64);
+        bad |= !(fabsf(v) < 65504.0f);
+        s2 += (double)v * (double)v;
+        s1 += fabs((double)v);
+    }
+    const double kappa = 1.02 * 0x1p-10 + 64.0 * 0x1p-23;
+    pq[2 * i] = (float)((kappa * sqrt(s2) + 0x1p-24 * 8.0) * (1.0 + 1e-6));
+    pq[2 * i + 1] = (float)((0x1p-24 * s1 + 0x1p-40) * (1.0 + 1e-6));
+    if (bad) atomicOr(flag, 1);
+}
+hipError_t launch_pack_dec_prune(const dal3_layer& L, float* dw1c, float* pq, uint32_t* ident, int32_t* flag, hipStream_t s) {
+    hipLaunchKernelGGL(pack_dec_prune_kernel, dim3(((DEC_NULL_K + 1) * 64 + 255) / 256), dim3(256), 0, s, L, dw1c, pq, ident, flag);
+    return hipGetLastError();
+}
+
+__global__ __launch_bounds__(512) void dec_plan_kernel(const float* __restrict__ gb, const uint32_t* __restrict__ prune,
+                                                       const float* __restrict__ pq, const int32_t* __restrict__ prn_flag,
+                                                       const int32_t* __restrict__ dec_flag, uint32_t* __restrict__ plan_k,
+                                                       float* __restrict__ plan_gbc, int32_t* __restrict__ plan_nch) {
+    __shared__ uint32_t s_k[DEC_PLAN_LD];
+    __shared__ uint32_t s_cnt[8];
+    const int64_t b = blockIdx.x;
+    const int k = threadIdx.x, lane = k & 63, wv = k >> 6;
+    const int ch = 32 * (k >> 5) + tile_chan((k & 31) >> 1, k & 1);
+    const float* gbb = gb + b * 512;
+    const uint32_t* pu = prune + b * 513;
+    const float g = gbb[ch];
+    const uint32_t key = pu[ch];
+    const float U = __uint_as_float(prune_unkey(key)), X = __uint_as_float(pu[512]);
+    float E = fmaf(X, pq[2 * ch], pq[2 * ch + 1]);
+    E = fmaf(fabsf(g), 0x1p-17f, E);
+    const float t = g + U;
+    E = fmaf(fabsf(g) + fabsf(U), 0x1p-22f, E);
+    E = fmaf(E, 0x1p-20f, E);
+    const bool flagged = *prn_flag == 0 && *dec_flag == 0 && key != 0u && t + E < 0.0f;
+    const uint64_t bal = __ballot(!flagged);
+    if (lane == 0) s_cnt[wv] = (uint32_t)__popcll(bal);
+    for (int i = k; i < DEC_PLAN_LD; i += 512) s_k[i] = DEC_NULL_K;
+    __syncthreads();
+    uint32_t below = 0, n_live = 0;
+    for (int i = 0; i < 8; ++i) {
+        below += i < wv ? s_cnt[i] : 0u;
+        n_live += s_cnt[i];
+    }
+    if (!flagged) s_k[below + (uint32_t)__popcll(bal & ((1ull << lane) - 1ull))] = (uint32_t)k;
+    __syncthreads();
+    const int nch = 512 - (int)n_live < DAL3_DEC_MIN_DEAD
+                        ? 0 : max(2, (((int)n_live + 31) / 32 + DAL3_DEC_PLAN_ROUND - 1) & ~(DAL3_DEC_PLAN_ROUND - 1));
+    if (k == 0) plan_nch[b] = nch;
+    for (int i = k; i < DEC_PLAN_LD; i += 512) plan_k[b * DEC_PLAN_LD + i] = s_k[i];
+    const int m = k & 31, hh = (m >> 2) & 1, r = (m & 3) + 4 * (m >> 3);
+    const uint32_t kk = s_k[32 * (k >> 5) + 2 * r + hh];
+    plan_gbc[b * 512 + k] = kk < DEC_NULL_K ? gbb[32 * (kk >> 5) + tile_chan((kk & 31) >> 1, kk & 1)] : -1.0f;
+}
+hipError_t launch_dec_plan(const InsSegW& w, const float* gb, const uint32_t* prune, int B, uint32_t* plan_k, float* plan_gbc,
+                           int32_t* plan_nch, hipStream_t s) {
+    hipLaunchKernelGGL(dec_plan_kernel, dim3((unsigned)B), dim3(512), 0, s, gb, prune, w.prn_pq, w.prn_flag, w.dec_flag, plan_k,
+                       plan_gbc, plan_nch);
     return hipGetLastError();
 }
 
diff --git a/3dal_pytorch_amd/csrc/dal3_pointmlp.hip b/3dal_pytorch_amd/csrc/dal3_pointmlp.hip
--- a/3dal_pytorch_amd/csrc/dal3_pointmlp.hip
+++ b/3dal_pytorch_amd/csrc/dal3_pointmlp.hip
@@ -1,4 +1,6 @@
 #include <stdlib.h>
+
+#include <type_traits>
 
 #include "dal3_device.h"
 #include "dal3_kernels.h"
@@ -75,8 +77,8 @@
 #ifndef DAL3_DEC_GROUP
 #define DAL3_DEC_GROUP 4
 #endif
-static_assert(DAL3_DEC_GROUP == 1 || DAL3_DEC_GROUP == 2 || DAL3_DEC_GROUP == 4 || DAL3_DEC_GROUP == 8,
-              "a group's rows fit the queue's 256, and the groups tile the 16 chunks");
+static_assert(DAL3_DEC_GROUP == 2 || DAL3_DEC_GROUP == 4 || DAL3_DEC_GROUP == 8,
+              "a group's rows fit the queue's 256; the chunk loop goes in pairs, and the last group may be shorter");
 static_assert(DAL3_PF == 8, "the compacted body's ring holds exactly one dconv1 chunk between two blocks");
 #ifdef DAL3_DEC_COUNT
 __device__ unsigned long long g_dec_count[12];
@@ -197,7 +199,9 @@
 template <int T, bool SP>
 __device__ __forceinline__ void ins_seg_decode_tile(const InsSegW& w, const BCN& pts, int c_in, int n_pts, int64_t b, int n0,
                                                     const float* __restrict__ gb, float* __restrict__ logits,
-                                                    uint8_t* __restrict__ mask, float* __restrict__ slab, int lane, int wave) {
+                                                    uint8_t* __restrict__ mask, float* __restrict__ slab, int lane, int wave,
+                                                    const uint32_t* __restrict__ pk = nullptr, const float* __restrict__ gbc = nullptr,
+                                                    int nch = 16) {
     const int h = lane >> 5;
     STAMP(0);
     WRing<DAL3_PF> ring;
@@ -208,15 +212,22 @@
     const int pt = lane & 31;
     __amdgpu_buffer_rsrc_t wc = ring.rsrc;
     constexpr int G = DAL3_DEC_GROUP;
-    constexpr int TRIP = SP && G > 2 ? G : 2;
+    constexpr int TRIP = SP ? G : 2;
     uint32_t m[TRIP] = {};
+    uint32_t kq[TRIP / 2] = {};
     uint32_t pend = 0;
     typedef uint32_t u32x2 __attribute__((ext_vector_type(2)));
     u32x2 pend_e = {0u, DEC_Q_ZERO * 32u};
     u32x2* kl = reinterpret_cast<u32x2*>(slab + DEC_G_LIST);
+    __amdgpu_buffer_rsrc_t wd1 = ring.rsrc;
+    const int row_pos = 2 * ((lane & 3) + 4 * ((lane & 31) >> 3)) + ((lane >> 2) & 1);
+    uint32_t kf = 0, kn = 0;
     if constexpr (SP) {
         wc = __builtin_amdgcn_make_buffer_rsrc(const_cast<float*>(w.dw2c), 0, 512 * 1024, 0x00020000);
+        wd1 = __builtin_amdgcn_make_buffer_rsrc(const_cast<float*>(w.dw1c), 0, (DEC_NULL_K + 1) * 256, 0x00020000);
         slab[DEC_Q_ZERO * 32 + pt] = 0.0f;
+        kf = pk[row_pos];
+        kn = pk[32 + row_pos];
     }
 #ifdef DAL3_DEC_COUNT
     uint32_t n_dense = 0, n_comp = 0, n_steps = 0, n_live = 0;
@@ -228,7 +239,30 @@
         load_points<2, T>(pts, b, n0, n_pts, c_in, in, lane);
         f32x16 x1[T][2];
         first_layer<2, 2, T>(w.w1, w.b1, in, x1, lane);
-        mlp_layer_ring<2, 2, T>(ring, w.b2, gb, bias, x1, x2, lane);
+        if constexpr (SP) {
+            f32x16 c2a[T], c2b[T];
+            c2a[0] = bias;
+            mma_block_ring<2, T>(ring, x1, c2a, [&](int i) {
+                if (i == 0) bias = tile_from_channels(w.b2 + 32, h);
+            });
+            c2b[0] = bias;
+#pragma unroll
+            for (int i = 0; i < 8; ++i) {
+                const f32x4 a = ring.slot[i];
+                ring.slot[i] = __builtin_bit_cast(f32x4, __builtin_amdgcn_raw_buffer_load_b128(wd1, kf * 256u + (uint32_t)h * 128u + 16u * i, 0, 0));
+#pragma unroll
+                for (int e = 0; e < 4; ++e) c2b[0] = mfma32(a[e], x1[0][i / 4][4 * (i % 4) + e], c2b[0]);
+                DAL3_SCHED_FENCE();
+                if (i == 0) bias = tile_from_channels(gbc, h);
+                x2[0][0][2 * i] = relu1(c2a[0][2 * i]);
+                x2[0][0][2 * i + 1] = relu1(c2a[0][2 * i + 1]);
+                DAL3_SCHED_FENCE();
+            }
+            x2[0][1] = relu16(c2b[0]);
+            kf = kn;
+        } else {
+            mlp_layer_ring<2, 2, T>(ring, w.b2, gb, bias, x1, x2, lane);
+        }
     }
 
     f32x16 a2[T][8];
@@ -267,8 +301,8 @@
         S.a0 = __builtin_bit_cast(f32x4, __builtin_amdgcn_raw_buffer_load_b128(wc, voff, 0, 0));
         S.a1 = __builtin_bit_cast(f32x4, __builtin_amdgcn_raw_buffer_load_b128(wc, voff + 16u, 0, 0));
     };
-    auto dconv2_group = [&](int c0, const uint32_t* mg) {
-        constexpr int NG = G;
+    auto dconv2_group = [&](auto ng, int c0, const uint32_t* mg) {
+        constexpr int NG = decltype(ng)::value;
         __builtin_amdgcn_fence(__ATOMIC_ACQ_REL, "wavefront");
         __builtin_amdgcn_wave_barrier();
         kl[0] = pend_e;
@@ -280,7 +314,7 @@
             const uint32_t word = h ? w1 : w0;
             if ((word >> pt) & 1u) {
                 u32x2 e;
-                e[0] = (32u * (uint32_t)(c0 + 2 * j) + (uint32_t)lane) * 1024u;
+                e[0] = kq[j] * 1024u;
                 e[1] = (64u * j + (uint32_t)lane) * 32u;
                 kl[total + below] = e;
             }
@@ -336,14 +370,10 @@
 #endif
     };
     auto dconv2_chunk = [&](const f32x16 (&t)[T], int c, int u) {
-        if constexpr (SP) {
-            if ((u + 1) % G == 0) dconv2_group(c + 1 - G, m + (u + 1 - G));
-        } else {
 #ifdef DAL3_DEC_COUNT
-            ++n_dense, n_live += 32;
-#endif
-            dconv2_part(t);
-        }
+        ++n_dense, n_live += 32;
+#endif
+        dconv2_part(t);
     };
     auto relu_note = [&](f32x16& t, int i, int u) {
         t[2 * i] = relu1(t[2 * i]);
@@ -363,9 +393,59 @@
             }
         }
     };
-    auto skip_dconv2 = [&]() {
-        if constexpr (SP) ring.soff += 32 * 1024;
+    auto dconv1_block = [&](f32x16& acc, int cn2, auto side) {
+        const uint32_t voff = kf * 256u + (uint32_t)h * 128u;
+#pragma unroll
+        for (int i = 0; i < 8; ++i) {
+            const f32x4 a = ring.slot[i];
+            ring.slot[i] = __builtin_bit_cast(f32x4, __builtin_amdgcn_raw_buffer_load_b128(wd1, voff + 16u * i, 0, 0));
+#pragma unroll
+            for (int e = 0; e < 4; ++e) acc = mfma32(a[e], x2[0][i / 4][4 * (i % 4) + e], acc);
+            DAL3_SCHED_FENCE();
+            if (i == 0) kn = pk[32 * cn2 + row_pos];
+            side(i);
+            DAL3_SCHED_FENCE();
+        }
+        kf = kn;
     };
+    if constexpr (SP) {
+        tA[0] = bias;
+        dconv1_block(tA[0], 2, [&](int i) {
+            if (i == 0) bias = tile_from_channels(gbc + 32, h);
+        });
+        auto pair = [&](int c, auto uc) {
+            constexpr int u = decltype(uc)::value;
+            tB[0] = bias;
+            dconv1_block(tB[0], c + 3, [&](int i) {
+                if (i == 0) bias = tile_from_channels(gbc + 32 * (c + 2 < nch ? c + 2 : 0), h);
+                if (i == 1) kq[(u / 2) % (TRIP / 2)] = pk[32 * c + lane];
+                relu_note(tA[0], i, u);
+            });
+            tA[0] = bias;
+            dconv1_block(tA[0], c + 4, [&](int i) {
+                if (i == 0) bias = c + 2 < nch ? tile_from_channels(gbc + 32 * (c + 3 < nch ? c + 3 : 0), h) : tile_from_channels(w.db3, h);
+                relu_note(tB[0], i, u + 1);
+            });
+        };
+        for (int c0 = 0; c0 < nch; c0 += G) {
+            bool done = false;
+#pragma unroll
+            for (int u = 0; u < G; u += 2) {
+                if (done) continue;
+                if (u == 0) pair(c0, std::integral_constant<int, 0>());
+                if (u == 2) pair(c0 + 2, std::integral_constant<int, 2>());
+                if (u == 4) pair(c0 + 4, std::integral_constant<int, 4>());
+                if (u == 6) pair(c0 + 6, std::integral_constant<int, 6>());
+                if (u + 2 < G && c0 + u + 2 >= nch) {
+                    if (u == 0) dconv2_group(std::integral_constant<int, 2>(), c0, m);
+                    if (u == 2) dconv2_group(std::integral_constant<int, 4>(), c0, m);
+                    if (u == 4) dconv2_group(std::integral_constant<int, 6>(), c0, m);
+                    done = true;
+                }
+            }
+            if (!done) dconv2_group(std::integral_constant<int, G>(), c0, m);
+        }
+    } else {
 #pragma unroll
     for (int j = 0; j < T; ++j) tA[j] = bias;
     mma_block_ring<2, T>(ring, x2, tA, [&](int i) {
@@ -377,7 +457,6 @@
             const int c = c0 + u;
 #pragma unroll
             for (int j = 0; j < T; ++j) tB[j] = bias;
-            skip_dconv2();
             mma_block_ring<2, T>(ring, x2, tB, [&](int i) {
                 if (i == 0) bias = tile_from_channels(gb + 32 * ((c + 2) & 15), h);
 #pragma unroll
@@ -386,7 +465,6 @@
             dconv2_chunk(tA, c, u);
 #pragma unroll
             for (int j = 0; j < T; ++j) tA[j] = bias;
-            skip_dconv2();
             mma_block_ring<2, T>(ring, x2, tA, [&](int i) {
                 if (i == 0)
                     bias = c + 2 < 16 ? tile_from_channels(gb + 32 * ((c + 3) & 15), h) : tile_from_channels(w.db3, h);
@@ -395,6 +473,7 @@
             });
             dconv2_chunk(tB, c + 1, u + 1);
         }
+    }
     }
     if constexpr (SP) {
         if (pend) {
@@ -488,7 +567,7 @@
 template <int T>
 __global__ __launch_bounds__(64 * DAL3_WG_WAVES) void ins_seg_decode_kernel(InsSegW w, BCN pts, int c_in, int n_pts,
                                                              int tiles_per_item, const float* __restrict__ gbias,
-                                                             float* __restrict__ logits, uint8_t* __restrict__ mask) {
+                                                             float* __restrict__ logits, uint8_t* __restrict__ mask, DecPlan plan) {
     const int lane = threadIdx.x & 63;
     const int wave = threadIdx.x >> 6;
 #ifndef DAL3_DEC_XCD
@@ -506,14 +585,23 @@
     constexpr bool SP = DAL3_DEC_SPARSE != 0 && T == 1;
     extern __shared__ __attribute__((aligned(16))) float s_slab[];
     if constexpr (SP) {
-        const f32x4 g0 = reinterpret_cast<const f32x4*>(gb)[2 * lane], g1 = reinterpret_cast<const f32x4*>(gb)[2 * lane + 1];
-        uint32_t neg = 0;
-#pragma unroll
-        for (int e = 0; e < 4; ++e)
-            neg += __builtin_popcountll(__builtin_amdgcn_ballot_w64(__float_as_int(g0[e]) < 0)) +
-                   __builtin_popcountll(__builtin_amdgcn_ballot_w64(__float_as_int(g1[e]) < 0));
-        if (neg >= DAL3_DEC_MIN_DEAD && *w.dec_flag == 0) {
-            ins_seg_decode_tile<T, true>(w, pts, c_in, n_pts, b, n0, gb, logits, mask, s_slab + wave * DEC_Q_FLOATS, lane, wave);
+        int nch = plan.nch ? plan.nch[b] : 0;
+        const uint32_t* pk = plan.k + b * DEC_PLAN_LD;
+        const float* gbc = plan.gbc + b * 512;
+        bool sparse = nch > 0;
+        if (!sparse) {
+            const f32x4 g0 = reinterpret_cast<const f32x4*>(gb)[2 * lane], g1 = reinterpret_cast<const f32x4*>(gb)[2 * lane + 1];
+            uint32_t neg = 0;
+#pragma unroll
+            for (int e = 0; e < 4; ++e)
+                neg += __builtin_popcountll(__builtin_amdgcn_ballot_w64(__float_as_int(g0[e]) < 0)) +
+                       __builtin_popcountll(__builtin_amdgcn_ballot_w64(__float_as_int(g1[e]) < 0));
+            sparse = neg >= DAL3_DEC_MIN_DEAD && *w.dec_flag == 0;
+            nch = 16, pk = w.dec_ident, gbc = gb;
+        }
+        if (sparse) {
+            ins_seg_decode_tile<T, true>(w, pts, c_in, n_pts, b, n0, gb, logits, mask, s_slab + wave * DEC_Q_FLOATS, lane, wave, pk,
+                                         gbc, nch);
             return;
         }
     }
@@ -704,7 +792,15 @@
 #endif
 bool lat_use(int64_t tiles, int flags, int64_t max_tiles) { return !(flags & DAL3_BCN_NO_SMALL_JOB_KERNELS) && tiles <= max_tiles; }
 
-hipError_t launch_ins_seg_encode(const InsSegW& w, BCN pts, int c_in, int B, int N, float* g, hipStream_t s) {
+bool dec_plan_route(int flags, int B, int N) {
+    const int64_t tiles = (int64_t)B * ((N + 31) / 32);
+    if (flags & DAL3_BCN_NO_DEC_PLAN) return false;
+    if (!DAL3_ENC_SCREEN || !DAL3_DEC_SPARSE || DAL3_DEC_T != 1) return false;
+    if (lat_use(tiles, flags, DAL3_LAT_MAX_TILES_ENC) || lat_use(tiles, flags, DAL3_LAT_MAX_TILES_DEC)) return false;
+    return !(DAL3_ENC_T > 1 && (int64_t)B * N <= 1024 * 64);
+}
+
+hipError_t launch_ins_seg_encode(const InsSegW& w, BCN pts, int c_in, int B, int N, float* g, hipStream_t s, uint32_t* prune) {
     if (lat_use((int64_t)B * ((N + 31) / 32), pts.flags, DAL3_LAT_MAX_TILES_ENC)) return launch_ins_seg_encode_lat(w, pts, c_in, B, N, g, s);
     constexpr int T = DAL3_ENC_T;
     if (T > 1 && (int64_t)B * N <= 1024 * 64) {
@@ -712,14 +808,14 @@
         hipLaunchKernelGGL(ins_seg_encode_kernel<1>, dim3((unsigned)((int64_t)B * tpi1)), dim3(64 * DAL3_WG_WAVES), 0, s, w, pts, c_in, N, tpi1, g);
         return hipGetLastError();
     }
-    if (DAL3_ENC_SCREEN) return launch_ins_seg_encode_screen(w, pts, c_in, B, N, g, s);
+    if (DAL3_ENC_SCREEN) return launch_ins_seg_encode_screen(w, pts, c_in, B, N, g, s, prune);
     const int tpi = tiles_per_item(N, T);
     hipLaunchKernelGGL(ins_seg_encode_kernel<T>, dim3((unsigned)((int64_t)B * tpi)), dim3(64 * DAL3_WG_WAVES), 0, s, w, pts, c_in, N, tpi, g);
     return hipGetLastError();
 }
 
 hipError_t launch_ins_seg_decode(const InsSegW& w, BCN pts, int c_in, int B, int N, const float* gbias,
-                                 float* logits, uint8_t* mask, hipStream_t s) {
+                                 float* logits, uint8_t* mask, hipStream_t s, DecPlan plan) {
     if (lat_use((int64_t)B * ((N + 31) / 32), pts.flags, DAL3_LAT_MAX_TILES_DEC)) return launch_ins_seg_decode_lat(w, pts, c_in, B, N, gbias, logits, mask, s);
     constexpr int T = DAL3_DEC_T;
     const int tpi = tiles_per_item(N, T);
@@ -730,7 +826,7 @@
         if (e != hipSuccess) return e;
     }
     hipLaunchKernelGGL(ins_seg_decode_kernel<T>, dim3((unsigned)((int64_t)B * tpi)), dim3(64 * DAL3_WG_WAVES), lds, s, w, pts, c_in, N, tpi,
-                       gbias, logits, mask);
+                       gbias, logits, mask, plan);
     return hipGetLastError();
 }
 
diff --git a/3dal_pytorch_amd/csrc/dal3_screen.h b/3dal_pytorch_amd/csrc/dal3_screen.h
--- a/3dal_pytorch_amd/csrc/dal3_screen.h
+++ b/3dal_pytorch_amd/csrc/dal3_screen.h
@@ -5,6 +5,9 @@
 __device__ __forceinline__ uint32_t scr_push_hit(uint32_t hb, float acc, float k) {
     return __builtin_amdgcn_alignbit(hb, __float_as_uint(k - acc), 31);
 }
+
+__host__ __device__ __forceinline__ uint32_t prune_key(uint32_t bits) { return bits ^ ((bits >> 31) ? 0xFFFFFFFFu : 0x80000000u); }
+__host__ __device__ __forceinline__ uint32_t prune_unkey(uint32_t key) { return key ^ ((key >> 31) ? 0x80000000u : 0xFFFFFFFFu); }
 
 template <int T>
 __host__ __device__ constexpr uint32_t scr_tile_mask(int j) {
diff --git a/include/dal3.h b/include/dal3.h
--- a/include/dal3.h
+++ b/include/dal3.h
@@ -64,9 +64,10 @@
     int32_t flags;
 } dal3_bcn;
 
-enum { DAL3_BCN_NO_SMALL_JOB_KERNELS = 1, DAL3_BCN_NO_WORKLIST = 2, DAL3_BCN_NO_LDS_SAMPLER = 4 };
+enum { DAL3_BCN_NO_SMALL_JOB_KERNELS = 1, DAL3_BCN_NO_WORKLIST = 2, DAL3_BCN_NO_LDS_SAMPLER = 4, DAL3_BCN_NO_DEC_PLAN = 16 };
 
 size_t dal3_ins_seg_workspace_bytes(int B);
+int dal3_ins_seg_plan_layout(int B, size_t off[4], int* min_dead);
 int dal3_ins_seg_forward(const void* packed, int dtype, int c_in, dal3_bcn pts, int B, int N,
                          float* logits, uint8_t* mask, float* global_feat_out,
                          void* workspace, size_t workspace_bytes, dal3_stream stream);
```

Result: faster. 243,400 object-crops/s, median of 6 (+4.1%).
